# ceres-solver/ceres-solver

Hardware: AMD Instinct MI355X
Metric: LM trust-region steps/sec (linear-solve hot path) + JtJx SpMV HBM GB/s on BAL (higher is better)
Workload: dtype f64; 1 GPU; venice1778-shaped synthetic BAL Jacobian <2,3,9>: 1778 cameras, 993923 points, 5001946 observations, N(0,1) values, seed 38401, camera popularity skew 0.6; solver=ITERATIVE_SCHUR + SCHUR_JACOBI, termination=SUCCESS, parallelism=1 GPU, inputs_resident_in_hbm=True, step_finite=True, jacobian_storage=fp64, camera_accumulators_in_lds=True

## Files before the change

### ceres-solver_amd/csrc/common.h

```cpp
#ifndef CERES_HIP_COMMON_H_
#define CERES_HIP_COMMON_H_

#include <cstdint>
#include <string>
#include <vector>

#include "../../include/ceres_hip.h"

namespace chip {

constexpr int kTile = 64;
constexpr int kMaxGenericBlock = 16;
constexpr int kCamChunk = 512;
constexpr int kPairsPerSlot = 12;
#ifndef CERES_HIP_AB_TILE_ROWS
#define CERES_HIP_AB_TILE_ROWS 12
#endif
constexpr int kTilePitch = CERES_HIP_AB_TILE_ROWS * 64;
constexpr size_t kLdsBytesPerCu = 160 * 1024;
constexpr int kSchurItem = 128;
constexpr int kZUnit = 64;
constexpr int kMaxPointsPerTile = 42;
constexpr int kSlotCamBits = 20;
constexpr int kSlotSpill = 0xFFF;
constexpr int kSlotNoCamera = (1 << kSlotCamBits) - 1;
constexpr int kPipelineMinTilesPerWg = 40;
constexpr int kStagedXMinTilesPerWg = 100;
constexpr int kCamItemLaneMinMean = 384;
constexpr int kCamItemSpread = 8192;
constexpr int kNonTemporalTileMiB = 200;

struct HostStructure {
  int nrb = 0, ncb = 0, nelim = 0, ncells = 0;
  std::vector<int32_t> rsz, rpos, csz, cpos, rptr, ccol, cval;
  int num_rows = 0, num_cols = 0, num_cols_e = 0, num_cols_f = 0, num_row_blocks_e = 0;
  int64_t nnz = 0;
  int64_t values_extent = 0;
  int max_block = 0;
  int det_row = 0, det_e = 0, det_f = 0;
  std::vector<int32_t> tptr, trow, tcell;
  std::vector<int32_t> row_block_of, col_block_of;
  std::vector<int64_t> diag_off_all;
  std::vector<int64_t> diag_off_f;
  std::vector<int64_t> diag_off_e;
  std::vector<int32_t> row_e_block;
  std::vector<int32_t> chunk_start, chunk_size;
  bool chunks_contiguous = true;
};

constexpr int kMaxSharedScalars = 8;
constexpr int kMaxSharedCellsPerRow = 2;
inline bool BalShapeCompiled(int nr, int ne, int nf, int ns) {
  if (nr == 3) return ne == 3 && nf == 3 && ns == 0;
  if (nr == 4) return ne == 4 && ns == 0 && (nf == 2 || nf == 3 || nf == 4);
  if (nr != 2) return false;
  if (ne == 2) return ns == 0 && (nf == 2 || nf == 3 || nf == 4 || nf == 6 || nf == 9);
  if (ne == 4) return ns == 0 && nf >= 2 && nf <= 10;
  if (ne != 3) return false;
  if (ns == 0) return nf >= 2 && nf <= 10;
  return (nf == 6 || nf == 9) && (ns == 4 || ns == 8);
}
inline int BalStripWidthFor(int ns_used) { return ns_used <= 0 ? 0 : (ns_used <= 4 ? 4 : (ns_used <= 8 ? 8 : -1)); }
// ... 102 lines not shown
```

### ceres-solver_amd/csrc/device.h

```cpp
#ifndef CERES_HIP_DEVICE_H_
#define CERES_HIP_DEVICE_H_

#include <hip/hip_runtime.h>

#include <cstdint>

#include "common.h"

namespace chip {

int BalBlockFor(int mode);
constexpr size_t kMaxLdsBytes = 160 * 1024;
constexpr int kVecBlock = 256;
constexpr int kMaxVecGrid = 512;
constexpr int kMaxEvalGrid = 2048;
constexpr int kMaxLsCameraGrid = 4096;

constexpr int kP2pMaxWorld = 8;
constexpr int kP2pChunk = 512;
constexpr int kP2pFlagChunk = 8;
constexpr int kP2pMaxGrid = 256;
struct P2pPeers {
  double* slots[kP2pMaxWorld];
  unsigned long long* flags[kP2pMaxWorld];
// ... 65 lines not shown
  const int32_t* d_pos = nullptr;
  double* D_int_out = nullptr;
  const double* x_e = nullptr;
  const double* x_f = nullptr;
  int flags = 0;
  double* y_e = nullptr;
  const double* D_e = nullptr;
  double lm_radius = 0.0, lm_min = 0.0, lm_max = 0.0;
  double* lm_diag_e = nullptr;
  double* lm_D_e = nullptr;
  double* etei = nullptr;
  double* point_blocks = nullptr;
  const int64_t* pt_diag_off = nullptr;
  double* Mo = nullptr;
  const int32_t* mo_index = nullptr;
  int have_b = 0;
  double* partials = nullptr;
  double* zbuf = nullptr;
  double* strip_sums = nullptr;
  int n_acc = 0;
  const int32_t* xhot_cam = nullptr;
  int n_xhot = 0;
  int x_lds_scalars = 0;
  double* scalar_out = nullptr;
  const double* copy_src = nullptr;
  double* copy_dst = nullptr;
  int copy_n = 0;
  int negate_out = 0;
  int* nonfinite = nullptr;
  const int* run_after_cg = nullptr;
  double* pq_out = nullptr;
  const int* status = nullptr;
  int* clear_flags = nullptr;
  CgTail tail;
};

struct LmFuse {
  double radius = 0.0, min_d = 0.0, max_d = 0.0;
  const double* camsq = nullptr;
  const int32_t* cam_pos = nullptr;
  int cam_base = 0;
  double* diag_f = nullptr;
  double* D_f = nullptr;
};

constexpr int kLossNone = -1, kLossTrivial = 0, kLossHuber = 1, kLossSoftLOne = 2, kLossCauchy = 3, kLossArctan = 4, kLossTolerant = 5,
              kLossTukey = 6;
struct LossParams {
  int32_t type = kLossNone;
  double a = 0.0, b = 0.0, c = 0.0, k = 1.0;
};

struct CamItems {
  const int32_t *cam = nullptr, *begin = nullptr, *end = nullptr;
  int count = 0;
  int64_t observations = 0;
  const double *ev_cam_pack = nullptr, *ev_pt_pack = nullptr;
  const int32_t* ev_pt = nullptr;
  const double2* ev_obs = nullptr;
  LossParams ev_loss;
};
struct CamGather {
  const double* parts = nullptr;
  const int32_t* cam_item_ptr = nullptr;
  const double* D_f = nullptr;
  const int32_t* cam_pos = nullptr;
  int cam_base = 0;
  int want_sq = 0;
  int few = 0;
  const double* extra = nullptr;
  const double* packed = nullptr;
};
struct ZUnits {
  const int32_t *cam = nullptr, *begin = nullptr, *end = nullptr, *shared = nullptr;
  const int32_t* slot = nullptr;
  int first = 0, count = 0;
};

struct FMap {
  const int32_t* cam_pos = nullptr;
  int cam_base = 0, n_cam_scalars = 0;
  int sh_pos[kMaxSharedScalars] = {};
};

struct StripBlocks {
  int count = 0;
  int off[kMaxSharedScalars] = {}, width[kMaxSharedScalars] = {}, pos[kMaxSharedScalars] = {};
  int64_t out[kMaxSharedScalars] = {};
};

struct BalOps {
  int nr, ne, nf, ns, pairs, tile_pitch, cam_part, etei_pitch, b_pairs, mo_pitch, has_f32, has_cg_tail;
  hipError_t (*fused)(int mode, const BalArgs& A, bool lds, int grid, hipStream_t stream);
  bool (*sx_runs_pipelined)(const BalArgs& A);
  hipError_t (*reduce_partials)(const double* partials, int nparts, int n_acc, const FMap& map, const double* D_f, const double* x_f,
                                double* y_f, const int* status, double* pq_out, int* n_pq, hipStream_t stream, const double* sum_in,
                                int n_sum_in, double* sum_out);
  hipError_t (*reduce_exchange)(const double* partials, int nparts, int n_acc, int n_fv, const FMap& map, const double* D_f, const double* x_f,
                                double* y_f, const int* status, double* pq_out, int* n_pq, hipStream_t stream, const double* sum_in,
                                int n_sum_in, double* sum_out, const P2pComm& comm, int grid_cap);
  hipError_t (*stream_probe)(const double2* J, int64_t n_tiles, int grid, double* out, hipStream_t stream);
  hipError_t (*add_f_diagonal)(int n_acc, const FMap& map, const double* D_f, const double* x_f, double* y_f, const int* status,
                               double* pq_out, int* n_pq, hipStream_t stream);
  hipError_t (*pack)(const BalArgs& A, hipStream_t stream);
  hipError_t (*invert)(double* blocks, const int64_t* cam_diag_off, int n_cameras, int* fail_flag, const LmFuse& lm, const CamGather& gather,
                       hipStream_t stream);
  hipError_t (*camera_exchange)(const double* parts, const int32_t* cam_item_ptr, int n_cameras, const double* extra, double* packed,
                                const P2pComm& comm, int grid_cap, hipStream_t stream, bool few );
  hipError_t (*camera_items)(bool schur, const double* values, const CamItems& items, const int32_t* cam_fpos, const int32_t* cam_slot,
                             const double* Mo, double* parts, hipStream_t stream);
  hipError_t (*camera_finish)(const double* parts, const int32_t* cam_item_ptr, const double* D_f, const int32_t* cam_pos, int cam_base,
                              const int64_t* cam_diag_off, double* blocks, double* camsq, int n_cameras, hipStream_t stream, const double* extra,
                              bool few );
  hipError_t (*camera_chunk)(const ZUnits& units, const double* ring, double* acc, const int* status, hipStream_t stream);
  hipError_t (*strip_finish)(const double* parts, int nparts, const StripBlocks& sb, const double* D_f, double* blocks, hipStream_t stream);
};
const BalOps* GetBalOps(int nr, int ne, int nf, int ns);
hipError_t AllowMaxLds(const void* kernel);

constexpr int kGenItem = 128;
constexpr int kGenItemValues = 55;
struct GenItems {
  int count = 0, first_block = 0, nblocks = 0;
  const int32_t *block = nullptr, *t0 = nullptr, *t1 = nullptr;
  const int32_t* block_ptr = nullptr;
  double* scratch = nullptr;
};
struct GenStructure {
  int nrb = 0, ncb = 0, nelim = 0, nrbe = 0, num_rows = 0, num_cols = 0, nce = 0, ncf = 0;
  const int32_t *rsz = nullptr, *rpos = nullptr, *rptr = nullptr, *ccol = nullptr, *cval = nullptr;
  const int32_t *csz = nullptr, *cpos = nullptr;
  const int32_t *tptr = nullptr, *trow = nullptr, *tcell = nullptr;
  const int32_t *tval = nullptr, *trpos = nullptr, *tinfo = nullptr;
  const int32_t *row_block_of = nullptr, *col_block_of = nullptr, *row_e_block = nullptr;
  const int64_t *diag_off_all = nullptr, *diag_off_e = nullptr, *diag_off_f = nullptr;
  const int32_t *chunk_start = nullptr, *chunk_size = nullptr;
  int max_csz_e = 0, max_csz_f = 0, max_csz = 0, max_rsz = 0;
  int lanes_e = 0, lanes_f = 0, lanes_all = 0, lanes_chunk = 0;
  GenItems items;
};
enum GenPart { kAll = 0, kE = 1, kF = 2 };

hipError_t LaunchGenRightMultiply(const GenStructure& G, const double* values, int part, const double* x, double* y,
                                  const int* status, hipStream_t stream);
hipError_t LaunchGenLeftMultiply(const GenStructure& G, const double* values, int part, const double* x, double* y,
                                 const int* status, hipStream_t stream);
hipError_t LaunchGenBlockDiagonal(const GenStructure& G, const double* values, int part, const double* D,
                                  double* blocks, int64_t total_entries, hipStream_t stream);
// ... 92 lines not shown
};
hipError_t LaunchCgnrModelCost(const double* y, const double* g, const double* r, const double* D, int64_t begin, int64_t end,
                               double* partials, int* nparts, hipStream_t stream, double* neg_out = nullptr, int* nonfinite = nullptr,
                               const int* gate = nullptr, const PointPerm& perm = PointPerm());
hipError_t LaunchPermutePoints(const double* in, double* out, const int32_t* pt_pos, int64_t n_e, int64_t n, bool to_internal, hipStream_t stream);
hipError_t LaunchNegateAndCheck(double* x, int64_t n, int* nonfinite, hipStream_t stream);
hipError_t LaunchGenScaleColumns(const GenStructure& G, double* values, const double* scale, hipStream_t stream);
hipError_t LaunchExpandSym(const double* packed, int ne, int pitch, double* dense, const int64_t* pt_diag_off, int n_points, hipStream_t stream);
hipError_t LaunchScatterBlocks9(const double* in, double* out, const int64_t* off, int n_points, hipStream_t stream);

enum CgStatus {
  kCgRunning = 0,
  kCgConvergedZeta = 1,
  kCgConvergedResidual = 2,
  kCgMaxIterations = 3,
  kCgFailRho = 4,
  kCgFailBeta = 5,
  kCgIndefinite = 6,
  kCgFailAlpha = 7,
  kCgZeroRhs = 8,
  kCgInitialResidual = 9,
  kCgSetupFailed = 10,
};
__host__ __device__ inline bool CgStatusAllowsSolution(int st) {
  return st != kCgRunning && st != kCgFailRho && st != kCgFailBeta && st != kCgFailAlpha && st != kCgSetupFailed;
}

struct CgScalars {
  double norm_rhs, tol_r, q_tol;
  double rho, rho_new, beta, pq, alpha, Q0, Q1, zeta, norm_r, norm_p, norm_q;
  int iter, status, min_it, max_it;
  int fail_dir, fail_step;
  double rho_pp[2], Q0_pp[2];
};

struct CgBuffers {
  int64_t n = 0;
  int64_t n_local = 0;
  int grid = 1, grid_e = 0;
  double *x = nullptr, *r = nullptr, *p = nullptr, *z = nullptr;
  const double* rhs = nullptr;
  double* partials = nullptr;
  double* comm = nullptr;
  CgScalars* S = nullptr;
  const int* setup_fail = nullptr;
  const double* pq_parts = nullptr;
  int n_pq = 0;
  const double* pq_extra = nullptr;
};
constexpr int kMaxPqParts = 2048;

hipError_t LaunchCgRhsNorm(const CgBuffers& B, hipStream_t stream);
hipError_t LaunchCgInit(const CgBuffers& B, double q_tol, double r_tol, int min_it, int max_it, hipStream_t stream);
hipError_t LaunchCgPrecondition(const CgBuffers& B, const GenStructure& G, int first_block, int col_begin, int nblocks,
                                int n_local_blocks, const int64_t* diag_off, const double* blocks, hipStream_t stream);
hipError_t LaunchCgDotSlot(const CgBuffers& B, const double* x, const double* y, int slot, hipStream_t stream);
hipError_t LaunchCgInitFromGuess(const CgBuffers& B, const double* tmp, double q_tol, double r_tol, int min_it, int max_it,
                                 hipStream_t stream);
hipError_t LaunchCgDirection(const CgBuffers& B, hipStream_t stream);
hipError_t LaunchCgDotPq(const CgBuffers& B, hipStream_t stream);
hipError_t LaunchCgStep(const CgBuffers& B, int reset, hipStream_t stream);
hipError_t LaunchCgResidualReset(const CgBuffers& B, const double* tmp, hipStream_t stream);
hipError_t LaunchCgFinalize(const CgBuffers& B, hipStream_t stream);
hipError_t LaunchCgUpdate(const CgBuffers& B, const GenStructure& G, int first_block, int col_begin, int nblocks,
                          const int64_t* diag_off, const double* blocks, int reset, int it, int nine_from, hipStream_t stream);
hipError_t LaunchCgBegin(const CgBuffers& B, double q_tol, double r_tol, int min_it, int max_it, hipStream_t stream);
hipError_t LaunchCgFinalizeDirection(const CgBuffers& B, int it, hipStream_t stream);
// ... 148 lines not shown
```

### ceres-solver_amd/csrc/kernels_bal.inc

```
#include <hip/hip_runtime.h>

#include <algorithm>
#include <mutex>
#include <unordered_map>

#include "device.h"
#include "p2p.h"
#ifndef CERES_HIP_NE
#define CERES_HIP_NE 3
#endif
#ifndef CERES_HIP_NR
#define CERES_HIP_NR 2
#endif
#if CERES_HIP_NE == 3 && CERES_HIP_NR == 2
#define CERES_HIP_PIPELINED 1
#else
#define CERES_HIP_PIPELINED 0
#endif
#if CERES_HIP_NR == 2 && CERES_HIP_NE == 3 && CERES_HIP_NF == 9 && CERES_HIP_NS == 0
#define CERES_HIP_IS_BAL_SHAPE 1
#include "robust_loss.h"
#include "snavely.h"
#else
#define CERES_HIP_IS_BAL_SHAPE 0
// ... 707 lines not shown
__device__ __forceinline__ void store_ete_inverse(const BalArgs& A, int pt, const double (&ei)[kTriE]) {
  if (A.etei) {
    double2* q = reinterpret_cast<double2*>(A.etei + int64_t(pt) * kEteiPitch);
#pragma unroll
    for (int j = 0; j < kEteiPitch / 2; ++j) tile_store<2>(q + j, make_double2(ei[2 * j], 2 * j + 1 < kTriE ? ei[(2 * j + 1) % kTriE] : 0.0));
  }
  if (A.point_blocks) {
    double* o = A.point_blocks + (A.pt_diag_off ? A.pt_diag_off[pt] : int64_t(NE * NE) * pt);
#pragma unroll
    for (int i = 0; i < NE; ++i) {
#pragma unroll
      for (int j = 0; j < NE; ++j) o[NE * i + j] = ei[i <= j ? tri_e(i, j) : tri_e(j, i)];
    }
  }
}

__device__ __forceinline__ void slot_point_sums(const Slot& s, double (&r)[kNX]) {
  double a[kTriE], g[NE];
  ete_of(s, a);
  et_times(s.e, s.b, g);
#pragma unroll
  for (int i = 0; i < kTriE; ++i) r[i] = s.valid ? a[i] : 0.0;
#pragma unroll
  for (int j = 0; j < NE; ++j) r[kTriE + j] = s.valid ? g[j] : 0.0;
}
__device__ __forceinline__ void store_point_solution(const BalArgs& A, int po, const double (&v)[NE]) {
  const double sg = A.negate_out ? -1.0 : 1.0;
  double t = 0.0;
#pragma unroll
  for (int j = 0; j < NE; ++j) { A.y_e[po + j] = sg * v[j]; t += v[j]; }
  if (A.negate_out && !isfinite(t)) atomicAdd(A.nonfinite, 1);
}

__device__ __forceinline__ double cost_terms(const double (&m)[NR], const double (&b)[NR], double half) {
  double t = 0.0;
#pragma unroll
  for (int r = 0; r < NR; ++r) t += m[r] * (b[r] + half * m[r]);
  return t;
}

template <bool LDS>
__device__ __forceinline__ void init_apply(const BalArgs& A, const Slot& s, int64_t sl,
                                           const double (&ei)[kTriE], const double (&g)[NE], Ctx& acc) {
  double h[NE], eh[NR], w[NR];
  sym_mul(ei, g, h);
  e_times(s.e, h, eh);
#pragma unroll
  for (int r = 0; r < NR; ++r) w[r] = s.b[r] - eh[r];
  if (A.have_b) scatter_ft<LDS>(A, s, acc, w);
  if (A.Mo && s.valid) {
    double q[NR][NE];
#pragma unroll
    for (int r = 0; r < NR; ++r) {
      double er[NE];
#pragma unroll
      for (int j = 0; j < NE; ++j) er[j] = s.e[r * NE + j];
      sym_mul(ei, er, q[r]);
    }
    double m[kMoPitch];
#pragma unroll
    for (int i = 0; i < kMoPitch; ++i) m[i] = 0.0;
#pragma unroll
    for (int a = 0; a < NR; ++a) {
#pragma unroll
      for (int b = 0; b < NR; ++b) {
        if (b < a) continue;
// ... 14 lines not shown
  double xc[NF];
  double ei[kTriE];
  double xa, xb, da, db;
  double xp[NE], dd[NE];
  int64_t base;
  bool coop;
};

template <int MODE>
__device__ __forceinline__ void load_aux(const BalArgs& A, const Slot& s, int lane, int npts, StreamAux& x) {
  load_xc(A, s.cam, x.xc);
  x.xa = x.xb = x.da = x.db = 0.0;
  x.base = 0;
  x.coop = false;
#pragma unroll
  for (int j = 0; j < NE; ++j) { x.xp[j] = 0.0; x.dd[j] = 0.0; }
  if constexpr (MODE == kSx || MODE == kSpseZ) {
    load_ete_inverse(A, s.pt, x.ei);
  } else if constexpr (MODE == kJtJx) {
    x.coop = CERES_HIP_PIPELINED && A.pt_pos == nullptr && !(A.flags & 1);
    if (x.coop) {
      const int n3 = 3 * npts;
      x.base = 3 * int64_t(__builtin_amdgcn_readfirstlane(s.pt));
      if (lane < n3) { x.xa = A.x_e[x.base + lane]; if (A.D_e) x.da = A.D_e[x.base + lane]; }
      if (n3 > 64 && lane + 64 < n3) { x.xb = A.x_e[x.base + 64 + lane]; if (A.D_e) x.db = A.D_e[x.base + 64 + lane]; }
    } else {
      const int po = pt_off(A, s.pt);
#pragma unroll
      for (int j = 0; j < NE; ++j) { x.xp[j] = A.x_e[po + j]; if (A.D_e) x.dd[j] = A.D_e[po + j]; }
    }
  }
}

template <int MODE, bool LDS>
__device__ __forceinline__ void compute_stream(const BalArgs& A, const Slot& s, int lane, int span, int npts,
                                               const StreamAux& x, Ctx& acc, double& dot) {
  if constexpr (MODE == kSx || MODE == kSpseZ) {
    double v[NE];
    double t[NR];
    f_times(s, acc, x.xc, t);
    double u[NE];
    et_times(s.e, t, u);
    if (!s.valid) {
#pragma unroll
      for (int j = 0; j < NE; ++j) u[j] = 0;
    }
#if !(CERES_HIP_AB_ABLATE & 4)
    seg_allreduce<NE>(u, lane, s.first, s.last, span);
#endif
    sym_mul(x.ei, u, v);
    double ev[NR], z[NR];
    e_times(s.e, v, ev);
#pragma unroll
    for (int r = 0; r < NR; ++r) z[r] = MODE == kSx ? t[r] - ev[r] : ev[r];
    scatter_ft<LDS>(A, s, acc, z);
  } else {
    static_assert(MODE == kJtJx, "streaming modes");
    double xp[NE];
#pragma unroll
    for (int j = 0; j < NE; ++j) xp[j] = x.xp[j];
#if CERES_HIP_PIPELINED
    const int n3 = 3 * npts;
    if (x.coop) {
      const int li = s.valid ? 3 * s.pt - int(x.base) : 0;
      if (n3 <= 64) {
#pragma unroll
        for (int j = 0; j < 3; ++j) xp[j] = shfl_idx(x.xa, li + j);
      } else {
#pragma unroll
        for (int j = 0; j < 3; ++j) {
          const double va = shfl_idx(x.xa, (li + j) & 63), vb = shfl_idx(x.xb, (li + j) & 63);
          xp[j] = (li + j) < 64 ? va : vb;
        }
      }
    }
#endif
    double z[NR];
    f_times(s, acc, x.xc, z);
    {
      double ex[NR];
      e_times(s.e, xp, ex);
#pragma unroll
// ... 154 lines not shown
    scatter_ft<LDS>(A, s, acc, s.b);
    double w[NE];
    et_times(s.e, s.b, w);
    if (!s.valid) {
#pragma unroll
      for (int j = 0; j < NE; ++j) w[j] = 0;
    }
    seg_scan<NE>(w, lane, s.first, span);
    if (s.valid && lane == s.last) {
#pragma unroll
      for (int j = 0; j < NE; ++j) A.y_e[po + j] = w[j];
    }
  } else if constexpr (MODE == kInit || MODE == kEte) {
    double r[kNX];
    slot_point_sums(s, r);
    if constexpr (MODE == kInit) {
      seg_allreduce<kNX>(r, lane, s.first, s.last, span);
    } else {
      double a6[kTriE];
#pragma unroll
      for (int i = 0; i < kTriE; ++i) a6[i] = r[i];
      seg_allreduce<kTriE>(a6, lane, s.first, s.last, span);
#pragma unroll
      for (int i = 0; i < kTriE; ++i) r[i] = a6[i];
    }
    double a[kTriE], ei[kTriE];
#pragma unroll
    for (int i = 0; i < kTriE; ++i) a[i] = r[i];
    add_e_diagonal(A, s.pt, po, a, s.valid && lane == s.last);
    if (!s.valid) set_identity_e(a);
    invert_spd_e(a, ei);
    if (s.valid && lane == s.last) store_ete_inverse(A, s.pt, ei);
    if constexpr (MODE == kInit) {
      double g[NE];
#pragma unroll
      for (int j = 0; j < NE; ++j) g[j] = r[kTriE + j];
      init_apply<LDS>(A, s, sl, ei, g, acc);
    }
  } else if constexpr (MODE == kColNorm) {
    double w[NE];
    e_col_squares(s, w);
    if (!s.valid) {
#pragma unroll
      for (int j = 0; j < NE; ++j) w[j] = 0;
    }
    scatter_f_squares(s, acc);
    seg_scan<NE>(w, lane, s.first, span);
    if (s.valid && lane == s.last) {
#pragma unroll
      for (int j = 0; j < NE; ++j) A.y_e[po + j] = w[j];
    }
  } else if constexpr (MODE == kJx) {
    double xc[NF];
    load_xc(A, s.cam, xc);
    double xe[NE];
#pragma unroll
    for (int j = 0; j < NE; ++j) xe[j] = A.x_e[po + j];
    double m[NR], ex[NR];
    f_times(s, acc, xc, m);
    e_times(s.e, xe, ex);
#pragma unroll
    for (int r = 0; r < NR; ++r) m[r] += ex[r];
    if (s.valid) lane_acc -= cost_terms(m, s.b, 0.5);
  } else if constexpr (MODE == kCgnrInit) {
    double r[kNX];
    slot_point_sums(s, r);
// ... 174 lines not shown
      }
    }
  } else if constexpr (MODE == kInit || MODE == kEte || MODE == kCgnrInit) {
    double r[kNX];
#pragma unroll
    for (int i = 0; i < kNX; ++i) r[i] = 0.0;
    int pt = 0;
    for (int t = 0; t < nt; ++t) {
      load_slot<kCanGather<MODE>, F32>(A, tile + t, lane, s, kWantsB<MODE>);
      if (t == 0) pt = __shfl(s.pt, 0, 64);
      if constexpr (MODE == kCgnrInit) scatter_ft<LDS>(A, s, acc, s.b);
      double q[kNX];
      slot_point_sums(s, q);
#pragma unroll
      for (int i = 0; i < kNX; ++i) r[i] += q[i];
    }
    wave_allreduce<kNX>(r);
    const int po = pt_off(A, pt);
    double a[kTriE], ei[kTriE];
#pragma unroll
    for (int i = 0; i < kTriE; ++i) a[i] = r[i];
    add_e_diagonal(A, pt, po, a, lane == 0);
    invert_spd_e(a, ei);
    if constexpr (MODE == kCgnrInit) {
      if (lane == 0) {
#pragma unroll
        for (int j = 0; j < NE; ++j) A.y_e[po + j] = r[kTriE + j];
        if (A.point_blocks) store_ete_inverse(A, pt, ei);
      }
    } else {
      if (lane == 0) store_ete_inverse(A, pt, ei);
    }
    if constexpr (MODE == kInit) {
      double g[NE];
#pragma unroll
      for (int j = 0; j < NE; ++j) g[j] = r[kTriE + j];
      for (int t = 0; t < nt; ++t) {
        load_slot<false, F32>(A, tile + t, lane, s, true, false);
        const int64_t sl = (tile + t) * kTile + lane;
        init_apply<LDS>(A, s, sl, ei, g, acc);
      }
    }
  }
}

template <int MODE, bool LDS, int BLOCK, bool F32>
__device__ __forceinline__ void fused_long_rounds(const BalArgs& A, int lane, bool grouped, int range, Ctx& acc, double& lane_acc) {
  constexpr int NX = (MODE == kInit || MODE == kEte || MODE == kCgnrInit) ? kNX : NE;
  constexpr int SUBS = BLOCK / 64 / kRoundWaves;
  constexpr bool kTwoPhase = (MODE == kSx || MODE == kSpseZ || MODE == kInit || MODE == kBackSub);
  static_assert(SUBS >= 1, "a workgroup holds at least one round");
  __shared__ double xr[SUBS][kRoundWaves][NX];
  const int wave_all = __builtin_amdgcn_readfirstlane(int(threadIdx.x >> 6));
  const int sub = wave_all / kRoundWaves, wave = wave_all % kRoundWaves;
  const int64_t qe = grouped ? int64_t(A.round_ptr[range + 1]) : int64_t(A.n_seq);
  const int64_t qstride = grouped ? 1 : int64_t(gridDim.x) * SUBS;
  const int64_t q_first = grouped ? int64_t(A.round_ptr[range]) : logical_workgroup() * SUBS;
  int64_t n_iter = 0;
  for (int j = 0; j < (grouped ? 1 : SUBS); ++j) {
    int64_t n = 0;
    if (grouped) { if (q_first < qe) n = A.seq_ptr[qe] - A.seq_ptr[q_first]; }
    else for (int64_t q = q_first + j; q < qe; q += qstride) n += A.seq_ptr[q + 1] - A.seq_ptr[q];
    n_iter = max(n_iter, n);
  }
  int64_t it_q = q_first + (grouped ? 0 : sub);
  bool it_real = grouped ? (sub == 0 && it_q < qe) : it_q < qe;
// ... 96 lines not shown
      }
    } else if (apply_round) {
#pragma unroll
      for (int i = 0; i < NX; ++i) tot[i] = carry[i];
      if (flag & kRoundLast) {
#pragma unroll
        for (int i = 0; i < NX; ++i) carry[i] = 0.0;
      }
      if constexpr (!kTwoPhase) continue;
    }
    if (!active) continue;
    const bool finish = wave == w0 && lane == 0 && !apply_round;
    const bool apply = flag == 0 || apply_round;
    if constexpr (MODE == kColNorm || MODE == kJtb) {
      if (finish) {
#pragma unroll
        for (int j = 0; j < NE; ++j) A.y_e[po + j] = tot[j];
      }
    } else if constexpr (MODE == kJtJx) {
      if (finish) {
#pragma unroll
        for (int j = 0; j < NE; ++j) {
          double d = 0;
          if (A.D_e) { d = A.D_e[po + j]; d = d * d * xp[j]; }
          A.y_e[po + j] = tot[j] + d;
          lane_acc += xp[j] * (tot[j] + d);
        }
      }
    } else if constexpr (MODE == kSx || MODE == kSpseZ || MODE == kBackSub) {
      double ei[kTriE], v[NE], u[NE];
      load_ete_inverse(A, pt, ei);
#pragma unroll
      for (int j = 0; j < NE; ++j) u[j] = tot[j];
      sym_mul(ei, u, v);
      if constexpr (MODE == kBackSub) {
        if (finish) store_point_solution(A, po, v);
        if (!A.scalar_out || !apply) continue;
      } else if (!apply) continue;
      if (apply_round) {
        double xc[NF];
        load_xc(A, s.cam, xc);
        f_times(s, acc, xc, ft);
        if constexpr (MODE == kBackSub) {
#pragma unroll
          for (int r = 0; r < NR; ++r) ft[r] = s.b[r] - ft[r];
        }
      }
      double ev[NR];
      e_times(s.e, v, ev);
      if constexpr (MODE == kBackSub) {
        double m[NR];
#pragma unroll
        for (int r = 0; r < NR; ++r) m[r] = (s.b[r] - ft[r]) + ev[r];
        if (s.valid) lane_acc += cost_terms(m, s.b, -0.5);
      } else {
        double z[NR];
#pragma unroll
        for (int r = 0; r < NR; ++r) z[r] = MODE == kSx ? ft[r] - ev[r] : ev[r];
        scatter_ft<LDS>(A, s, acc, z);
      }
    } else {
      double a[kTriE], ei[kTriE];
#pragma unroll
      for (int i = 0; i < kTriE; ++i) a[i] = tot[i];
      add_e_diagonal(A, pt, po, a, finish);
      invert_spd_e(a, ei);
      if constexpr (MODE == kCgnrInit) {
        if (finish) {
#pragma unroll
          for (int j = 0; j < NE; ++j) A.y_e[po + j] = tot[kTriE + j];
          if (A.point_blocks) store_ete_inverse(A, pt, ei);
        }
      } else {
        if (finish) store_ete_inverse(A, pt, ei);
      }
      if constexpr (MODE == kInit) {
        if (apply) {
          double g[NE];
#pragma unroll
          for (int j = 0; j < NE; ++j) g[j] = tot[kTriE + j];
          init_apply<LDS>(A, s, tile * kTile + lane, ei, g, acc);
        }
      }
    }
  }
}

template <int MODE, bool LDS, int BLOCK, bool F32>
__global__ __launch_bounds__(BLOCK) void bal_fused_kernel(BalArgs A) {
  extern __shared__ double lds_acc[];
  if constexpr (MODE == kInit || MODE == kCgnrInit) {
    if (A.clear_flags && blockIdx.x == 0 && threadIdx.x == 0) { A.clear_flags[0] = 0; A.clear_flags[1] = 0; }
  }
  if (A.status && *A.status != 0) return;
  if (A.run_after_cg && !CgStatusAllowsSolution(*A.run_after_cg)) return;
  constexpr bool kScatters = (MODE == kSx || MODE == kJtJx || MODE == kJtb || MODE == kInit || MODE == kCgnrInit || MODE == kColNorm || MODE == kSpseZ);
  Ctx acc;
  ctx_init(A, acc, nullptr);
  if constexpr (kScatters) {
    acc.lds = lds_acc;
    const int n_acc = LDS ? A.n_acc : NF * A.hyb_rows;
    for (int i = threadIdx.x; i < n_acc; i += BLOCK) acc.lds[i] = 0.0;
    __syncthreads();
  }
  if constexpr (MODE == kBackSub || MODE == kJx) {
    if (A.x_lds_scalars > 0) {
      for (int i = threadIdx.x; i < A.x_lds_scalars; i += BLOCK) lds_acc[i] = A.x_f[cam_off(A, i / NF) + i % NF];
      __syncthreads();
    }
  }
  const int lane = threadIdx.x & 63;
  double lane_acc = 0.0;
  if constexpr (MODE == kBackSub) {
    if (A.copy_dst)
      for (int i = blockIdx.x * BLOCK + threadIdx.x; i < A.copy_n; i += gridDim.x * BLOCK) {
        const double z = A.copy_src[i];
        A.copy_dst[i] = A.negate_out ? -z : z;
        if (A.negate_out && !isfinite(z)) atomicAdd(A.nonfinite, 1);
      }
  }
  const bool grouped = kScatters && !LDS && A.grp_tile_ptr != nullptr;
  const int64_t tile0 = grouped ? A.grp_tile_ptr[blockIdx.x] + (threadIdx.x >> 6) : A.tile_begin + logical_workgroup() * (BLOCK / 64) + (threadIdx.x >> 6);
  const int64_t nwaves = grouped ? BLOCK / 64 : int64_t(gridDim.x) * (BLOCK / 64);
  const int64_t tile_end = grouped ? A.grp_tile_ptr[blockIdx.x + 1] : (A.tile_end > 0 ? A.tile_end : A.n_tiles);
  if constexpr (MODE == kShBlocks) {
    for (int64_t tile = tile0; tile < tile_end; tile += nwaves) {
      const int kind = A.tile_kind[tile];
      const int aux = A.tile_aux[tile];
// ... 208 lines not shown
      const int w = sp + j * ns;
      v[j] = (mine && w < nparts) ? A.partials[int64_t(w) * n + i] : 0.0;
    }
#pragma unroll
    for (int h = kCgTailLoads / 2; h >= 1; h >>= 1) {
#pragma unroll
      for (int j = 0; j < h; ++j) v[j] += v[j + h];
    }
    if (mine) part[idx] = v[0];
  }
  __syncthreads();
  double qv[PER];
  double pq = 0, unused0 = 0, unused1 = 0;
#pragma unroll
  for (int k = 0; k < PER; ++k) {
    const int i = threadIdx.x + k * BLOCK;
    qv[k] = 0.0;
    if (i < n) {
      double q = 0;
      for (int sp = 0; sp < ns; ++sp) q += part[sp * n + i];
      q += dv[k] * dv[k] * pv[k];
      qv[k] = q;
      pq += pv[k] * q;
    }
  }
  sum3(pq, unused0, unused1);
  if (staged) pq = 1.0;
  int fail = staged;
  double alpha = 0;
  if (!fail) {
    if (pq <= 0 || isinf(pq)) fail = kCgIndefinite;
    else { alpha = rho / pq; if (isinf(alpha)) fail = kCgFailAlpha; }
  }
  if (threadIdx.x == 0) { S.pq = pq; S.alpha = alpha; S.rho_new = rho; S.fail_step = fail; }
  if (fail) {
    if (threadIdx.x == 0) S.status = fail;
    return;
  }
  double q1 = 0, rr = 0, rz = 0, rn[PER], zv[PER];
#pragma unroll
  for (int k = 0; k < PER; ++k) {
    const int i = threadIdx.x + k * BLOCK;
    rn[k] = 0.0;
    if (i < n) {
      const double xv = xo[k] + alpha * pv[k];
      const double rv = ro[k] - alpha * qv[k];
      T.x[i] = xv; T.r[i] = rv;
      rn[k] = rv;
      lds[i] = rv;
      q1 -= xv * (bv[k] + rv);
      rr += rv * rv;
    }
  }
  __syncthreads();
#pragma unroll
  for (int k = 0; k < PER; ++k) {
    const int i = threadIdx.x + k * BLOCK;
    zv[k] = 0.0;
    if (i < n) {
      const int c = i / 9;
      double t = 0;
#pragma unroll
      for (int j = 0; j < 9; ++j) t += mrow[k][j] * lds[9 * c + j];
      zv[k] = t;
      T.z[i] = t;
      rz += rn[k] * t;
    }
// ... 3 lines not shown
  const double norm_r = sqrt(rr);
  const double zeta = it * (Q1 - Q0) / Q1;
  int status = kCgRunning;
  if (zeta < q_tol && it >= min_it) status = kCgConvergedZeta;
  else if (norm_r <= tol_r && it >= min_it) status = kCgConvergedResidual;
  else if (it >= max_it) status = kCgMaxIterations;
  int fail_dir = 0;
  double beta = 0.0;
  if (status == kCgRunning) {
    auto zero_or_inf = [](double v) { return v == 0.0 || isinf(v); };
    if (zero_or_inf(rho_next)) fail_dir = kCgFailRho;
    else { beta = rho_next / rho; if (zero_or_inf(beta)) fail_dir = kCgFailBeta; }
    if (!fail_dir) {
#pragma unroll
      for (int k = 0; k < PER; ++k) {
        const int i = threadIdx.x + k * BLOCK;
        if (i < n) T.p[i] = zv[k] + beta * pv[k];
      }
    }
  }
  if (threadIdx.x == 0) {
    S.Q1 = Q1; S.zeta = zeta; S.norm_r = norm_r;
    if (status == kCgConvergedZeta) { S.status = status; return; }
    S.Q0 = Q1;
    S.Q0_pp[(it + 1) & 1] = Q1;
    if (status != kCgRunning) { S.status = status; return; }
    S.rho = rho; S.rho_new = rho_next; S.beta = beta;
    S.rho_pp[(it + 1) & 1] = rho_next;
    S.fail_dir = fail_dir;
    S.iter = it + 1;
  }
}

template <int MODE, bool LDS>
__device__ __forceinline__ void compute_long_round(const BalArgs& A, const Slot& s, int lane, const StreamAux& x, uint32_t word, uint32_t word0,
                                                   int flag, int wave, double (*red)[3], double (&carry)[3], Ctx& acc, double& dot) {
  const bool active = word != kRoundIdle;
  const int w0 = flag ? 0 : (active ? int((word >> 26) & 7u) : wave);
  const int cnt = flag ? int((word0 >> 29) & 7u) + 1 : (active ? int((word >> 29) & 7u) + 1 : 1);
  if constexpr (MODE == kSx || MODE == kSpseZ) {
    double t0, t1;
    f_times(s, acc, x.xc, t0, t1);
    double u[3] = {s.e[0] * t0 + s.e[3] * t1, s.e[1] * t0 + s.e[4] * t1, s.e[2] * t0 + s.e[5] * t1};
    if (!s.valid) { u[0] = u[1] = u[2] = 0; }
    if (!(flag & kRoundApply)) {
      wave_allreduce<3>(u);
      if (lane == 0) { red[wave][0] = u[0]; red[wave][1] = u[1]; red[wave][2] = u[2]; }
    }
    __syncthreads();
    if (flag & kRoundApply) {
      u[0] = carry[0]; u[1] = carry[1]; u[2] = carry[2];
      if (flag & kRoundLast) { carry[0] = carry[1] = carry[2] = 0; }
    } else {
      u[0] = u[1] = u[2] = 0;
      for (int k = 0; k < cnt; ++k) { u[0] += red[w0 + k][0]; u[1] += red[w0 + k][1]; u[2] += red[w0 + k][2]; }
      if (flag & kRoundSum) { carry[0] += u[0]; carry[1] += u[1]; carry[2] += u[2]; return; }
    }
    double v[3];
    sym_mul(x.ei, u, v);
    const double ev0 = s.e[0] * v[0] + s.e[1] * v[1] + s.e[2] * v[2];
    const double ev1 = s.e[3] * v[0] + s.e[4] * v[1] + s.e[5] * v[2];
    scatter_ft<LDS>(A, s, acc, MODE == kSx ? t0 - ev0 : ev0, MODE == kSx ? t1 - ev1 : ev1);
  } else {
    static_assert(MODE == kJtJx, "streaming modes");
    if (flag & kRoundApply) { __syncthreads(); return; }
    const double xp[3] = {shfl_idx(x.xa, 0), shfl_idx(x.xa, 1), shfl_idx(x.xa, 2)};
    double z0, z1;
    f_times(s, acc, x.xc, z0, z1);
    z0 += s.e[0] * xp[0] + s.e[1] * xp[1] + s.e[2] * xp[2];
    z1 += s.e[3] * xp[0] + s.e[4] * xp[1] + s.e[5] * xp[2];
    scatter_ft<LDS>(A, s, acc, z0, z1);
    double w[3] = {s.e[0] * z0 + s.e[3] * z1, s.e[1] * z0 + s.e[4] * z1, s.e[2] * z0 + s.e[5] * z1};
    if (!s.valid) { w[0] = w[1] = w[2] = 0; }
    wave_allreduce<3>(w);
    if (lane == 0) { red[wave][0] = w[0]; red[wave][1] = w[1]; red[wave][2] = w[2]; }
    __syncthreads();
    double t = 0;
    if (lane < 3) {
      for (int k = 0; k < cnt; ++k) t += red[w0 + k][lane];
    }
    bool store = active && wave == w0 && lane < 3;
    if (flag & kRoundSum) {
      const double c = (lane == 0 ? carry[0] : (lane == 1 ? carry[1] : carry[2])) + t;
      if (lane == 0) carry[0] = c; else if (lane == 1) carry[1] = c; else if (lane == 2) carry[2] = c;
      store = store && (flag & kRoundLast);
      t = c;
      if (flag & kRoundLast) { carry[0] = carry[1] = carry[2] = 0; }
    }
    if (store) {
      const double yv = t + x.da * x.da * x.xa;
      A.y_e[x.base + lane] = yv;
      dot += x.xa * yv;
    }
  }
}

template <int MODE, bool LDS, bool NT, bool F32 = false>
__global__ __launch_bounds__(512) void bal_stream_kernel(BalArgs A) {
  constexpr int BLOCK = 512;
  extern __shared__ double lds_acc[];
  if (A.status && *A.status != 0) return;
  Ctx acc;
  ctx_init(A, acc, lds_acc);
  double* const xh = lds_acc + A.n_acc;
  {
    const int n_acc = LDS ? A.n_acc : NF * A.hyb_rows;
    for (int i = threadIdx.x; i < n_acc; i += BLOCK) acc.lds[i] = 0.0;
    if constexpr (LDS) {
      const int nx = NF * A.n_xhot;
      for (int i0 = threadIdx.x; i0 < nx; i0 += 4 * BLOCK) {
        int c[4];
        double v[4];
#pragma unroll
        for (int j = 0; j < 4; ++j) { const int i = i0 + j * BLOCK; c[j] = A.xhot_cam[(i < nx ? i : 0) / NF]; }
#pragma unroll
        for (int j = 0; j < 4; ++j) { const int i = i0 + j * BLOCK; v[j] = A.x_f[A.cam_base + NF * int64_t(c[j]) + (i < nx ? i : 0) % NF]; }
#pragma unroll
        for (int j = 0; j < 4; ++j) { const int i = i0 + j * BLOCK; if (i < nx) xh[i] = v[j]; }
      }
    }
    __syncthreads();
  }
  const int lane = threadIdx.x & 63;
  double dot = 0.0;
  const bool grouped = !LDS && A.grp_tile_ptr != nullptr;
  const int64_t nwaves = grouped ? BLOCK / 64 : int64_t(gridDim.x) * (BLOCK / 64);
  const int wave = __builtin_amdgcn_readfirstlane(int(threadIdx.x >> 6));
  const int range = grouped ? int(blockIdx.x) : 0;
  const int64_t range_end = grouped ? A.grp_tile_ptr[blockIdx.x + 1] : (A.tile_end > 0 ? A.tile_end : A.n_tiles);
  const int64_t long_begin = A.long_behind ? int64_t(A.long_ptr[range]) : range_end;
// ... 19 lines not shown
    issue_idx(A, t1, lane, i2);
    __builtin_amdgcn_sched_barrier(0);
    issue_idx(A, t2, lane, i1);
    __builtin_amdgcn_sched_barrier(0);
    issue_pairs<NT, F32>(A, tile, lane, sa);
    __builtin_amdgcn_sched_barrier(0);
    sa.cam = i0.cam; sa.seg = i0.seg;
    finish_slot(sa, lane, A.tile_pt0[tile]);
    issue_aux<MODE>(A, sa, lane, kind_a == 0 ? aux_a >> 8 : 0, xa);
    __builtin_amdgcn_sched_barrier(0);
    issue_pairs<NT, F32>(A, t1, lane, sb);
    __builtin_amdgcn_sched_barrier(0);
    sb.cam = i2.cam; sb.seg = i2.seg;
    finish_slot(sb, lane, A.tile_pt0[t1]);
    issue_aux<MODE>(A, sb, lane, kind_b == 0 ? aux_b >> 8 : 0, xb);
    __builtin_amdgcn_sched_barrier(0);
    bool more = true;
    auto stage = [&](Slot& c, StreamAux& cx, int ckind, int caux, Slot& f, StreamAux& fx, int& fkind, int& faux) {
      const int64_t far = min(tile + 2 * pstep, last);
      more = tile + pstep < pipe_end;
      fkind = A.tile_kind[far];
      faux = A.tile_aux[far];
      issue_idx(A, min(far + pstep, last), lane, i2);
      __builtin_amdgcn_sched_barrier(0);
      issue_pairs<NT, F32>(A, far, lane, f);
      __builtin_amdgcn_sched_barrier(0);
      f.cam = i1.cam; f.seg = i1.seg;
      finish_slot(f, lane, A.tile_pt0[far]);
      issue_aux<MODE>(A, f, lane, fkind == 0 ? faux >> 8 : 0, fx);
      __builtin_amdgcn_sched_barrier(0);
      if (ckind != 0) c.valid = false;
      widen_slot<F32>(c);
      if constexpr (LDS) take_hot_x(A, c, xh, cx);
      compute_stream<MODE, LDS>(A, c, lane, caux & 0xff, ckind == 0 ? caux >> 8 : 0, cx, acc, dot);
      __builtin_amdgcn_sched_barrier(0);
      i1 = i2;
      tile = min(tile + pstep, last);
    };
    while (true) {
      stage(sa, xa, kind_a, aux_a, sc, xc, kind_c, aux_c);
      if (!more) break;
      stage(sb, xb, kind_b, aux_b, sa, xa, kind_a, aux_a);
      if (!more) break;
      stage(sc, xc, kind_c, aux_c, sb, xb, kind_b, aux_b);
      if (!more) break;
    }
  }
#else
  if (pipe0 < pipe_end) {
    Slot sa, sb;
    StreamAux xa, xb;
    SlotIdx i1, i2;
    int64_t tile = pipe0;
    int kind_a = A.tile_kind[tile], aux_a = A.tile_aux[tile], kind_b = 2, aux_b = 0;
    issue_idx(A, tile, lane, i2);
    __builtin_amdgcn_sched_barrier(0);
    issue_idx(A, min(tile + pstep, last), lane, i1);
    __builtin_amdgcn_sched_barrier(0);
    issue_pairs<NT, F32>(A, tile, lane, sa);
    __builtin_amdgcn_sched_barrier(0);
    sa.cam = i2.cam; sa.seg = i2.seg;
    finish_slot(sa, lane, A.tile_pt0[tile]);
    issue_aux<MODE>(A, sa, lane, kind_a == 0 ? aux_a >> 8 : 0, xa);
    __builtin_amdgcn_sched_barrier(0);
    bool more = true;
    auto stage = [&](Slot& c, StreamAux& cx, int ckind, int caux, Slot& n, StreamAux& nx, int& nkind, int& naux) {
      const int64_t next = min(tile + pstep, last);
      more = tile + pstep < pipe_end;
#if CERES_HIP_AB_ABLATE & 16
      nkind = 0;
      naux = (13 << 8) | 8;
      const int npt0 = int(next) * 13;
#else
      nkind = A.tile_kind[next];
      naux = A.tile_aux[next];
      const int npt0 = A.tile_pt0[next];
#endif
      issue_idx(A, min(next + pstep, last), lane, i2);
      __builtin_amdgcn_sched_barrier(0);
      issue_pairs<NT, F32>(A, next, lane, n);
      __builtin_amdgcn_sched_barrier(0);
      n.cam = i1.cam; n.seg = i1.seg;
      finish_slot(n, lane, npt0);
      issue_aux<MODE>(A, n, lane, nkind == 0 ? naux >> 8 : 0, nx);
      __builtin_amdgcn_sched_barrier(0);
      if (ckind != 0) c.valid = false;
      widen_slot<F32>(c);
      if constexpr (LDS) take_hot_x(A, c, xh, cx);
      compute_stream<MODE, LDS>(A, c, lane, caux & 0xff, ckind == 0 ? caux >> 8 : 0, cx, acc, dot);
      __builtin_amdgcn_sched_barrier(0);
      i1 = i2;
      tile = next;
    };
    while (true) {
      stage(sa, xa, kind_a, aux_a, sb, xb, kind_b, aux_b);
      if (!more) break;
      stage(sb, xb, kind_b, aux_b, sa, xa, kind_a, aux_a);
      if (!more) break;
    }
  }
#endif
  __shared__ double round_red[2][kRoundWaves][3];
  if (A.round_word) {
    const int64_t qe = grouped ? int64_t(A.round_ptr[range + 1]) : int64_t(A.n_seq);
    const int64_t qstride = grouped ? 1 : int64_t(gridDim.x);
    int64_t it_q = grouped ? int64_t(A.round_ptr[range]) : logical_workgroup();
    if (it_q < qe) {
      int64_t it_r = A.seq_ptr[it_q], it_end = A.seq_ptr[grouped ? qe : it_q + 1];
      if (grouped) it_q = qe - 1;
      bool it_real = true;
      auto next_round = [&](bool* real) {
        const int64_t r = it_r;
        *real = it_real;
        if (it_real) {
          if (it_r + 1 < it_end) ++it_r;
          else if (it_q + qstride < qe) { it_q += qstride; it_r = A.seq_ptr[it_q]; it_end = A.seq_ptr[it_q + 1]; }
          else it_real = false;
        }
        return r;
      };
      Slot sa, sb;
      StreamAux xa, xb;
// ... 9 lines not shown
      bool real_c, real_n, real_nn;
      int64_t rc = next_round(&real_c), rn = next_round(&real_n);
      uint32_t wa = word_at(rc), wb = kRoundIdle;
      uint32_t w0a = A.round_word[rc * kRoundWaves], w0b = kRoundIdle;
      int fa = A.round_flag[rc], fb = 0;
      int par = 0;
      {
        const int64_t tile = tile_at(rc, wa);
        issue_idx(A, tile, lane, i2);
        __builtin_amdgcn_sched_barrier(0);
        issue_idx(A, tile_at(rn, word_at(rn)), lane, i1);
        __builtin_amdgcn_sched_barrier(0);
        issue_pairs<NT, F32>(A, tile, lane, sa);
        __builtin_amdgcn_sched_barrier(0);
        finish(sa, i2, tile, wa);
        issue_aux<MODE>(A, sa, lane, 1, xa);
        __builtin_amdgcn_sched_barrier(0);
      }
      auto stage = [&](Slot& c, StreamAux& cx, uint32_t cw, uint32_t cw0, int cf, Slot& n, StreamAux& nx, uint32_t& nw, uint32_t& nw0, int& nf) {
        const int64_t rnn = next_round(&real_nn);
        nw = word_at(rn);
        nw0 = A.round_word[rn * kRoundWaves];
        nf = A.round_flag[rn];
        const int64_t next = int64_t((nw != kRoundIdle ? nw : nw0) & 0x3FFFFFFu);
        issue_idx(A, tile_at(rnn, word_at(rnn)), lane, i2);
        __builtin_amdgcn_sched_barrier(0);
        issue_pairs<NT, F32>(A, next, lane, n);
        __builtin_amdgcn_sched_barrier(0);
        finish(n, i1, next, nw);
        issue_aux<MODE>(A, n, lane, 1, nx);
        __builtin_amdgcn_sched_barrier(0);
        widen_slot<F32>(c);
        if constexpr (LDS) take_hot_x(A, c, xh, cx);
        compute_long_round<MODE, LDS>(A, c, lane, cx, cw, cw0, cf, wave, round_red[par], carry, acc, dot);
        __builtin_amdgcn_sched_barrier(0);
        par ^= 1;
        i1 = i2;
        rc = rn; real_c = real_n;
        rn = rnn; real_n = real_nn;
      };
      while (true) {
        stage(sa, xa, wa, w0a, fa, sb, xb, wb, w0b, fb);
        if (!real_c) break;
        stage(sb, xb, wb, w0b, fb, sa, xa, wa, w0a, fa);
        if (!real_c) break;
      }
    }
  }
  for (int64_t tile = (A.long_behind ? long_begin + wave_first : wave0); tile < range_end; tile += nwaves) {
    if (A.tile_kind[tile] == 1) process_long_point<MODE, LDS, F32>(A, tile, A.tile_aux[tile], lane, acc, dot);
  }
  if (MODE == kJtJx && A.pq_out) {
    __shared__ double red[BLOCK / 64];
#pragma unroll
    for (int m = 32; m >= 1; m >>= 1) dot += __shfl_xor(dot, m, 64);
    if (lane == 0) red[threadIdx.x >> 6] = dot;
    __syncthreads();
    if (threadIdx.x == 0) {
      double t = 0;
      for (int i = 0; i < BLOCK / 64; ++i) t += red[i];
      if (A.pq_accumulate) t += A.pq_out[blockIdx.x];
      A.pq_out[blockIdx.x] = t;
    }
  }
  if constexpr (LDS) {
    flush_shared_sums(A, acc);
    __syncthreads();
// ... 830 lines not shown
  }
}

__global__ __launch_bounds__(1024) void bal_strip_finish_kernel(const double* __restrict__ parts, int nparts, StripBlocks sb,
                                                                const double* __restrict__ D_f, double* __restrict__ blocks) {
  __shared__ double T[16][kTriSX];
  const int lane = threadIdx.x & 63, wv = threadIdx.x >> 6;
  for (int i = lane; i < kTriS; i += 64) {
    double t0 = 0, t1 = 0;
    int w = wv;
    for (; w + 16 < nparts; w += 32) { t0 += parts[int64_t(w) * kTriS + i]; t1 += parts[int64_t(w + 16) * kTriS + i]; }
    if (w < nparts) t0 += parts[int64_t(w) * kTriS + i];
    T[wv][i] = t0 + t1;
  }
  __syncthreads();
  for (int i = threadIdx.x; i < kTriS; i += 1024) {
    double t = T[0][i];
    for (int w = 1; w < 16; ++w) t += T[w][i];
    T[0][i] = t;
  }
  __syncthreads();
  for (int q = 0; q < sb.count; ++q) {
    const int w = sb.width[q], o = sb.off[q];
    for (int e = threadIdx.x; e < w * w; e += 1024) {
      const int a = e / w, b = e - a * w;
      const int lo = o + (a < b ? a : b), hi = o + (a < b ? b : a);
      double v = T[0][lo * (2 * NS + 1 - lo) / 2 + (hi - lo)];
      if (a == b && D_f) { const double d = D_f[sb.pos[q] + a]; v += d * d; }
      blocks[sb.out[q] + e] = v;
    }
  }
}

}

template <int MODE, int BLOCK, bool F32>
static hipError_t launch_fused2(const BalArgs& A, bool lds, int grid, hipStream_t stream) {
  if (lds) {
    const size_t bytes = size_t(A.n_acc) * sizeof(double);
    auto k = bal_fused_kernel<MODE, true, BLOCK, F32>;
    if (hipError_t e = AllowMaxLds(reinterpret_cast<const void*>(k)); e != hipSuccess) return e;
    hipLaunchKernelGGL(k, dim3(grid), dim3(BLOCK), bytes, stream, A);
  } else {
    constexpr bool kScatters = (MODE == kSx || MODE == kJtJx || MODE == kJtb || MODE == kInit || MODE == kCgnrInit || MODE == kColNorm || MODE == kSpseZ);
    const size_t bytes = kScatters ? (size_t(A.hyb_rows) * NF + size_t(BLOCK / 64) * kTile * NF) * sizeof(double)
                                   : ((MODE == kBackSub || MODE == kJx) ? size_t(A.x_lds_scalars) * sizeof(double) : 0);
    auto k = bal_fused_kernel<MODE, false, BLOCK, F32>;
    if (bytes > 0)
      if (hipError_t e = AllowMaxLds(reinterpret_cast<const void*>(k)); e != hipSuccess) return e;
    hipLaunchKernelGGL(k, dim3(grid), dim3(BLOCK), bytes, stream, A);
  }
  return hipGetLastError();
}
template <int MODE, int BLOCK>
static hipError_t launch_fused(const BalArgs& A, bool lds, int grid, hipStream_t stream) {
  if constexpr (kHasF32) {
    if (A.Jf) return launch_fused2<MODE, BLOCK, true>(A, lds, grid, stream);
  } else {
    if (A.Jf) return hipErrorInvalidValue;
  }
  return launch_fused2<MODE, BLOCK, false>(A, lds, grid, stream);
}

#if CERES_HIP_PIPELINED
template <int MODE, bool NT, bool F32 = false>
static hipError_t launch_stream2(const BalArgs& A, bool lds, int grid, hipStream_t stream) {
  if (lds) {
    auto k = bal_stream_kernel<MODE, true, NT, F32>;
    if (hipError_t e = AllowMaxLds(reinterpret_cast<const void*>(k)); e != hipSuccess) return e;
    const size_t tail_bytes = (kHasCgTail && MODE == kSx && A.tail.enabled) ? size_t(512 + kCgTailMax) * sizeof(double) : 0;
    static const size_t static_lds = [&] { hipFuncAttributes fa{}; return hipFuncGetAttributes(&fa, reinterpret_cast<const void*>(k)) == hipSuccess ? size_t(fa.sharedSizeBytes) : size_t(1024); }();
    BalArgs B = A;
    if (size_t(B.n_acc) * sizeof(double) + size_t(B.n_xhot) * NF * sizeof(double) + static_lds > kMaxLdsBytes) B.n_xhot = 0;
    const size_t xhot_bytes = size_t(B.n_xhot) * NF * sizeof(double);
    hipLaunchKernelGGL(k, dim3(grid), dim3(512), size_t(B.n_acc) * sizeof(double) + std::max(tail_bytes, xhot_bytes), stream, B);
  } else {
    auto k = bal_stream_kernel<MODE, false, NT, F32>;
    if (hipError_t e = AllowMaxLds(reinterpret_cast<const void*>(k)); e != hipSuccess) return e;
    hipLaunchKernelGGL(k, dim3(grid), dim3(512), (size_t(A.hyb_rows) * NF + size_t(512 / 64) * kTile * NF) * sizeof(double), stream, A);
  }
  return hipGetLastError();
}
template <int MODE>
static hipError_t launch_stream(const BalArgs& A, bool lds, int grid, hipStream_t stream) {
  if (A.Jf) {
    if constexpr (kHasF32) {
      const bool nt32 = A.n_tiles * int64_t(6 * kTile) * int64_t(sizeof(float4)) > (int64_t(kNonTemporalTileMiB) << 20);
      return nt32 ? launch_stream2<MODE, true, true>(A, lds, grid, stream) : launch_stream2<MODE, false, true>(A, lds, grid, stream);
    } else {
      return hipErrorInvalidValue;
    }
  }
  const bool nt = A.n_tiles * int64_t(kTilePitch) * int64_t(sizeof(double2)) > (int64_t(kNonTemporalTileMiB) << 20);
  return nt ? launch_stream2<MODE, true>(A, lds, grid, stream) : launch_stream2<MODE, false>(A, lds, grid, stream);
}

#endif

static bool UsePipeline() {
  static int v = [] { const char* e = getenv("CERES_HIP_PIPELINE"); return e ? atoi(e) : 1; }();
  return CERES_HIP_PIPELINED && v != 0;
}

static bool F32Pipelined() {
  static int v = [] { const char* e = getenv("CERES_HIP_F32_PIPELINE"); return e ? atoi(e) : 1; }();
  return kHasF32 && v != 0;
}
static bool SxRunsPipelined(const BalArgs& A) { return UsePipeline() && (!A.Jf || F32Pipelined()) && !A.src_values && !A.cam_pos && !(A.flags & 1); }

static hipError_t Fused(int mode, const BalArgs& A0, bool lds, int grid, hipStream_t stream) {
  BalArgs A = A0;
  if ((mode != kBackSub && mode != kJx) || lds) A.x_lds_scalars = 0;
  if ((A.tile_end > 0 ? A.tile_end - A.tile_begin : A.n_tiles) < int64_t(kStagedXMinTilesPerWg) * grid) { A.n_xhot = 0; A.x_lds_scalars = 0; }
  const bool big = BalBlockFor(mode) == 1024;
  const bool few_tiles = (A.tile_end > 0 ? A.tile_end - A.tile_begin : A.n_tiles) < int64_t(kPipelineMinTilesPerWg) * grid && !A.tail.enabled && lds;
  const bool big_s = big && (lds || A.hyb_rows == 0) && !few_tiles;
#if CERES_HIP_PIPELINED
  if (UsePipeline() && !few_tiles && (!A.Jf || F32Pipelined()) && !A.src_values && !A.cam_pos && !(A.flags & 1)) {
    if (mode == kSx) return launch_stream<kSx>(A, lds, grid, stream);
    if (mode == kJtJx && A.D_e && !A.pt_pos) return launch_stream<kJtJx>(A, lds, grid, stream);
    if (mode == kSpseZ) return launch_stream<kSpseZ>(A, lds, grid, stream);
  }
#endif
  switch (mode) {
    case kSx: return big_s ? launch_fused<kSx, 1024>(A, lds, grid, stream) : launch_fused<kSx, 512>(A, lds, grid, stream);
    case kJtJx: return big_s ? launch_fused<kJtJx, 1024>(A, lds, grid, stream) : launch_fused<kJtJx, 512>(A, lds, grid, stream);
// ... 114 lines not shown
  static const int forced = [] { const char* e = getenv("CERES_HIP_CAM_ITEMS_MFMA"); return e ? (atoi(e) != 0 ? 1 : 0) : -1; }();
  const bool mfma = NR == 2 && (forced >= 0 ? forced == 1 : items.observations < int64_t(kCamItemLaneMinMean) * items.count);
  if (mfma) {
#if CERES_HIP_NR == 2
    if (schur) hipLaunchKernelGGL((bal_camera_items_mfma_kernel<true>), grid, dim3(256), 0, stream, values, items, cam_fpos, cam_slot, Mo, parts);
    else hipLaunchKernelGGL((bal_camera_items_mfma_kernel<false>), grid, dim3(256), 0, stream, values, items, cam_fpos, cam_slot, Mo, parts);
#endif
  } else {
    if (schur) hipLaunchKernelGGL((bal_camera_items_kernel<true>), grid, dim3(256), 0, stream, values, items, cam_fpos, cam_slot, Mo, parts);
    else hipLaunchKernelGGL((bal_camera_items_kernel<false>), grid, dim3(256), 0, stream, values, items, cam_fpos, cam_slot, Mo, parts);
  }
  return hipGetLastError();
}

static hipError_t CameraFinish(const double* parts, const int32_t* cam_item_ptr, const double* D_f, const int32_t* cam_pos, int cam_base,
                               const int64_t* cam_diag_off, double* blocks, double* camsq, int n_cameras, hipStream_t stream, const double* extra, bool few) {
  if (n_cameras > 0 && !few) {
    hipLaunchKernelGGL(bal_camera_finish_wide_kernel, dim3(n_cameras), dim3(64 * kInvertGatherWaves), 0, stream, parts, cam_item_ptr, D_f, cam_pos,
                       cam_base, cam_diag_off, blocks, camsq, n_cameras, extra);
    return hipGetLastError();
  }
  if (n_cameras > 0) hipLaunchKernelGGL(bal_camera_finish_kernel, dim3((n_cameras + kPerWave - 1) / kPerWave), dim3(64), 0, stream, parts, cam_item_ptr, D_f, cam_pos,
                                        cam_base, cam_diag_off, blocks, camsq, n_cameras, extra);
  return hipGetLastError();
}

static hipError_t CameraChunk(const ZUnits& units, const double* ring, double* acc, const int* status, hipStream_t stream) {
  if (units.count == 0) return hipSuccess;
  const int waves = (units.count + kPerWave - 1) / kPerWave;
  hipLaunchKernelGGL(bal_camera_chunk_kernel, dim3((waves + 3) / 4), dim3(256), 0, stream, units, ring, acc, status);
  return hipGetLastError();
}

}

#define CERES_HIP_CAT2(a, b) a##b
#define CERES_HIP_CAT(a, b) CERES_HIP_CAT2(a, b)
const BalOps* CERES_HIP_CAT(BalOps_, CERES_HIP_SHAPE)() {
  namespace sh = CERES_HIP_SHAPE;
  static const BalOps ops = {sh::NR, sh::NE, sh::NF, sh::NS, sh::kPairs, sh::kTilePitch, sh::kCamPart, sh::kEteiPitch, sh::kBPairs, sh::kMoPitch, sh::kHasF32 ? 1 : 0, sh::kHasCgTail ? 1 : 0,
                             sh::Fused, sh::SxRunsPipelined, sh::ReducePartials, sh::ReduceExchange, sh::StreamProbe, sh::AddFDiagonal, sh::Pack, sh::Invert, sh::CameraExchange,
                             sh::CameraItems, sh::CameraFinish, sh::CameraChunk, sh::StripFinish};
  return &ops;
}

}
```

### ceres-solver_amd/csrc/kernels_cg.hip

```cpp
#include <hip/hip_runtime.h>

#include <algorithm>

#include "device.h"
#include "p2p.h"

namespace chip {

namespace {

__device__ __forceinline__ double wave_sum(double v) {
#pragma unroll
  for (int m = 32; m >= 1; m >>= 1) v += __shfl_xor(v, m, 64);
  return v;
}

__device__ __forceinline__ double block_sum(double v, double* sh ) {
  v = wave_sum(v);
  __syncthreads();
  if ((threadIdx.x & 63) == 0) sh[threadIdx.x >> 6] = v;
  __syncthreads();
  return (sh[0] + sh[1]) + (sh[2] + sh[3]);
}

// ... 109 lines not shown
    const bool pt = perm.pt_pos && i < perm.n_e;
    const double yi = y[i], d = D ? (pt ? perm.D_e[i] : D[i]) * yi : 0.0;
    v += yi * (g[i] + r[i]) + d * d;
    if (neg_out) { neg_out[pt ? perm.pt_pos[i / 3] + int(i % 3) : i] = -yi; if (!isfinite(yi)) ++bad; }
  }
  if (bad) atomicAdd(nonfinite, bad);
  v = block_sum(v, sh);
  if (threadIdx.x == 0) partials[blockIdx.x] = v;
}

__global__ __launch_bounds__(kVecBlock) void cg_rhs_norm_kernel(CgBuffers B) {
  __shared__ double sh[4];
  double v = 0;
  for (Span s = my_span(B); s.i < s.end; s.i += s.step) v += B.rhs[s.i] * B.rhs[s.i];
  v = block_sum(v, sh);
  if (threadIdx.x == 0) B.partials[blockIdx.x] = v;
}

__global__ __launch_bounds__(kVecBlock) void cg_init_kernel(CgBuffers B, double q_tol, double r_tol, int min_it, int max_it) {
  __shared__ double sh[4];
  const double nn = total_of(B, 0, sh);
  for (Span s = my_span(B); s.i < s.end; s.i += s.step) { B.x[s.i] = 0.0; B.r[s.i] = B.rhs[s.i]; }
  if (blockIdx.x == 0 && threadIdx.x == 0) {
    CgScalars& S = *B.S;
    S.norm_rhs = sqrt(nn);
    S.tol_r = r_tol * S.norm_rhs;
    S.q_tol = q_tol;
    S.rho = 1.0; S.rho_new = 1.0; S.beta = 0; S.pq = 0; S.alpha = 0;
    S.Q0 = 0.0;
    S.Q0_pp[0] = 0.0; S.Q0_pp[1] = 0.0; S.rho_pp[0] = 1.0; S.rho_pp[1] = 1.0;
    S.Q1 = 0; S.zeta = 0; S.norm_r = S.norm_rhs; S.norm_p = 0; S.norm_q = 0;
    S.iter = 1; S.min_it = min_it; S.max_it = max_it;
    S.status = kCgRunning;
    S.fail_dir = 0; S.fail_step = 0;
    if (S.norm_rhs == 0.0) S.status = kCgZeroRhs;
    else if (min_it == 0 && S.norm_r <= S.tol_r) S.status = kCgInitialResidual;
    if (B.setup_fail && *B.setup_fail != 0) S.status = kCgSetupFailed;
  }
}

__global__ __launch_bounds__(kVecBlock) void cg_dot_slot_kernel(CgBuffers B, const double* x, const double* y, int slot) {
  __shared__ double sh[4];
  if (B.S->status != 0) return;
  double v = 0;
  for (Span s = my_span(B); s.i < s.end; s.i += s.step) v += x[s.i] * y[s.i];
  v = block_sum(v, sh);
  if (threadIdx.x == 0) B.partials[slot * kMaxVecGrid + blockIdx.x] = v;
}

__global__ __launch_bounds__(kVecBlock) void cg_init_from_guess_kernel(CgBuffers B, const double* tmp) {
  __shared__ double sh[4];
  double q = 0, rr = 0;
  for (Span s = my_span(B); s.i < s.end; s.i += s.step) {
    const double r = B.rhs[s.i] - tmp[s.i];
    B.r[s.i] = r;
    q -= B.x[s.i] * (B.rhs[s.i] + r);
    rr += r * r;
  }
  q = block_sum(q, sh);
  rr = block_sum(rr, sh);
  if (threadIdx.x == 0) { B.partials[2 * kMaxVecGrid + blockIdx.x] = q; B.partials[3 * kMaxVecGrid + blockIdx.x] = rr; }
}
__global__ __launch_bounds__(kVecBlock) void cg_init_from_guess_finish_kernel(CgBuffers B, double q_tol, double r_tol, int min_it, int max_it) {
  __shared__ double sh[4];
  const double nn = total_of(B, 0, sh);
  const double Q0 = total_of(B, 2, sh);
  const double rr = total_of(B, 3, sh);
  if (threadIdx.x != 0) return;
  CgScalars& S = *B.S;
  S.norm_rhs = sqrt(nn);
  S.tol_r = r_tol * S.norm_rhs;
  S.q_tol = q_tol;
  S.rho = 1.0; S.rho_new = 1.0; S.beta = 0; S.pq = 0; S.alpha = 0;
  S.Q0 = Q0; S.Q1 = 0; S.zeta = 0; S.norm_r = sqrt(rr); S.norm_p = 0; S.norm_q = 0;
  S.Q0_pp[0] = Q0; S.Q0_pp[1] = Q0; S.rho_pp[0] = 1.0; S.rho_pp[1] = 1.0;
  S.iter = 1; S.min_it = min_it; S.max_it = max_it;
  S.status = kCgRunning;
  S.fail_dir = 0; S.fail_step = 0;
  if (S.norm_rhs == 0.0) S.status = kCgZeroRhs;
  else if (min_it == 0 && S.norm_r <= S.tol_r) S.status = kCgInitialResidual;
  if (B.setup_fail && *B.setup_fail != 0) S.status = kCgSetupFailed;
}

template <int N>
__device__ __forceinline__ double precondition_block(const double* __restrict__ m, const double* __restrict__ r, double* __restrict__ z) {
  double rr[N], v = 0;
#pragma unroll
  for (int c = 0; c < N; ++c) rr[c] = r[c];
#pragma unroll
  for (int a = 0; a < N; ++a) {
    double s = 0;
#pragma unroll
    for (int c = 0; c < N; ++c) s += m[a * N + c] * rr[c];
    z[a] = s;
    v += rr[a] * s;
  }
  return v;
}

__global__ __launch_bounds__(kVecBlock) void cg_precondition_kernel(CgBuffers B, GenStructure G, int first_block, int col_begin,
                                                                    int nblocks, int n_local_blocks,
                                                                    const int64_t* diag_off, const double* blocks) {
  __shared__ double sh[4];
  if (B.S->status != 0) return;
  double v = 0;
  if (!blocks) {
    for (Span s = my_span(B); s.i < s.end; s.i += s.step) { const double r = B.r[s.i]; B.z[s.i] = r; v += r * r; }
  } else {
    int64_t q, q_end, q_step;
    if (int(blockIdx.x) < B.grid_e) {
      q = int64_t(blockIdx.x) * kVecBlock + threadIdx.x; q_end = n_local_blocks; q_step = int64_t(B.grid_e) * kVecBlock;
// ... 232 lines not shown
        else if (n == 9) update_block<9, START>(m, alpha, B.p + pos, B.rhs + pos, B.x + pos, B.r + pos, B.z + pos, q1, rr, rz);
        else {
          double rn[kMaxGenericBlock];
          for (int c = 0; c < n; ++c) {
            const double xv = START ? 0.0 : B.x[pos + c] + alpha * B.p[pos + c];
            const double rv = START ? B.rhs[pos + c] : B.r[pos + c] - alpha * B.z[pos + c];
            B.x[pos + c] = xv; B.r[pos + c] = rv; rn[c] = rv;
            q1 -= xv * (B.rhs[pos + c] + rv);
            rr += rv * rv;
          }
          for (int a = 0; a < n; ++a) {
            double t = 0;
            for (int c = 0; c < n; ++c) t += m[a * n + c] * rn[c];
            B.z[pos + a] = t;
            rz += rn[a] * t;
          }
        }
      }
    }
  }
  if (!reset) {
    block_sum3(q1, rr, rz, sh);
    if (threadIdx.x == 0) {
      B.partials[2 * kMaxVecGrid + blockIdx.x] = q1;
      B.partials[3 * kMaxVecGrid + blockIdx.x] = rr;
      B.partials[0 * kMaxVecGrid + blockIdx.x] = rz;
    }
  }
  if (!START && blockIdx.x == 0 && threadIdx.x == 0) {
    S.pq = pq;
    S.alpha = alpha;
    S.rho_new = rho;
    S.fail_step = fail;
  }
}

__global__ __launch_bounds__(kVecBlock) void cg_begin_kernel(CgBuffers B, double q_tol, double r_tol, int min_it, int max_it) {
  __shared__ double sh[12];
  double nn = 0, rho = 0, unused = 0;
  for (int k = B.grid_e + threadIdx.x; k < B.grid; k += kVecBlock) { nn += B.partials[3 * kMaxVecGrid + k]; rho += B.partials[0 * kMaxVecGrid + k]; }
  block_sum3(nn, rho, unused, sh);
  if (B.grid_e > 0) { nn += B.comm[3]; rho += B.comm[0]; }
  const double norm_rhs = sqrt(nn);
  const double tol_r = r_tol * norm_rhs;
  int status = kCgRunning;
  if (norm_rhs == 0.0) status = kCgZeroRhs;
  else if (min_it == 0 && norm_rhs <= tol_r) status = kCgInitialResidual;
  if (B.setup_fail && *B.setup_fail != 0) status = kCgSetupFailed;
  int fail_dir = 0;
  if (status == kCgRunning) {
    if (zero_or_inf(rho)) fail_dir = kCgFailRho;
    else
      for (int64_t i = int64_t(blockIdx.x) * kVecBlock + threadIdx.x; i < B.n; i += int64_t(gridDim.x) * kVecBlock) B.p[i] = B.z[i];
  }
  if (blockIdx.x == 0 && threadIdx.x == 0) {
    CgScalars& S = *B.S;
    S.norm_rhs = norm_rhs; S.tol_r = tol_r; S.q_tol = q_tol;
    S.rho = 1.0; S.rho_new = rho; S.beta = 0; S.pq = 0; S.alpha = 0;
    S.Q0 = 0.0; S.Q1 = 0; S.zeta = 0; S.norm_r = norm_rhs; S.norm_p = 0; S.norm_q = 0;
    S.Q0_pp[0] = 0.0; S.Q0_pp[1] = 0.0; S.rho_pp[0] = 1.0; S.rho_pp[1] = rho;
    S.iter = 1; S.min_it = min_it; S.max_it = max_it;
    S.fail_dir = fail_dir; S.fail_step = 0;
    S.status = status;
  }
}

__global__ __launch_bounds__(kVecBlock) void cg_finalize_direction_kernel(CgBuffers B, int it) {
  __shared__ double sh[12];
  CgScalars& S = *B.S;
  if (S.status != 0) return;
  const int fail = S.fail_step;
  if (fail != 0) {
    if (blockIdx.x == 0 && threadIdx.x == 0) S.status = fail;
    return;
  }
  double Q1 = 0, rr = 0, rho = 0;
  for (int k = B.grid_e + threadIdx.x; k < B.grid; k += kVecBlock) {
    Q1 += B.partials[2 * kMaxVecGrid + k];
    rr += B.partials[3 * kMaxVecGrid + k];
    rho += B.partials[0 * kMaxVecGrid + k];
  }
  block_sum3(Q1, rr, rho, sh);
  if (B.grid_e > 0) { Q1 += B.comm[2]; rr += B.comm[3]; rho += B.comm[0]; }
  const double Q0 = S.Q0_pp[it & 1], rho_prev = S.rho_pp[it & 1];
  const double norm_r = sqrt(rr);
  const double zeta = it * (Q1 - Q0) / Q1;
  int status = kCgRunning;
  if (zeta < S.q_tol && it >= S.min_it) status = kCgConvergedZeta;
  else if (norm_r <= S.tol_r && it >= S.min_it) status = kCgConvergedResidual;
  else if (it >= S.max_it) status = kCgMaxIterations;
  int fail_dir = 0;
  double beta = 0.0;
  if (status == kCgRunning) {
    if (zero_or_inf(rho)) fail_dir = kCgFailRho;
    else { beta = rho / rho_prev; if (zero_or_inf(beta)) fail_dir = kCgFailBeta; }
// ... 282 lines not shown
```

### ceres-solver_amd/csrc/solver.hip

```cpp
#include <hip/hip_runtime.h>
#include <rccl/rccl.h>

#include <exception>
#include <new>
#include <algorithm>
#include <chrono>
#include <climits>
#include <cmath>
#include <complex>
#include <cstdarg>
#include <cstdio>
#include <cstring>
#include <functional>
#include <limits>
#include <memory>
#include <mutex>
#include <numeric>
#include <sstream>
#include <string>
#include <type_traits>
#include <vector>

#include "device.h"

// ... 41 lines not shown
  uint32_t* d_slot_seg = nullptr;
  int32_t *d_tile_kind = nullptr, *d_tile_aux = nullptr, *d_pt_pos = nullptr, *d_cam_pos = nullptr;
  int32_t *d_cam_ptr = nullptr, *d_cam_fpos = nullptr, *d_cam_slot = nullptr;
  int32_t *d_tile_zbase = nullptr, *d_grp_tile_ptr = nullptr;
  unsigned int* d_cg_ticket = nullptr;
  bool cg_tail_enabled = [] { const char* e = getenv("CERES_HIP_CG_TAIL"); return !e || atoi(e) != 0; }();
  bool cam_exchange_few = false;
  bool cam_items_few = false;
  int32_t *d_long_ptr = nullptr, *d_round_ptr = nullptr, *d_seq_ptr = nullptr, *d_round_flag = nullptr;
  uint32_t* d_round_word = nullptr;
  int32_t* d_mo_index = nullptr;
  CamItems cam_items;
  int32_t* d_cam_item_ptr = nullptr;
  double* d_cam_parts = nullptr;
  double* d_cam_packed = nullptr;
  ZUnits zunits;
  int chunk_grid = 0;
  double *lm_diag = nullptr, *lm_D = nullptr, *scalar_partials = nullptr;
  int* d_nonfinite = nullptr;
  bool clear_flags_pending = false;
  bool fail_flag_clean = false, nonfinite_clean = false;
  bool have_lm_diag = false;
  bool lm_want_model_cost = false;
  bool lm_skip_model_cost = false;
  bool lm_negate_in_solve = false;
  bool lm_negated = false;
  bool lm_cgnr_copy_pending = false;
  bool speculate = true;
  bool lm_speculate = false;
  bool gate_on_cg_status = false;
  bool spec_tail_done = false;
  int spec_cgnr_parts = 0;
  int backsub_cost_parts = 0;
  bool lm_fuse_active = false;
  ceres_hip_lm_options lm_opts{};
  double* d_camsq = nullptr;
  int64_t *d_pt_diag_off = nullptr, *d_cam_diag_off = nullptr;
  int64_t* d_pt_eoff = nullptr;
  double2 *d_J = nullptr, *d_bt = nullptr;
  float4* d_Jf = nullptr;
  double *d_Mo = nullptr, *d_partials = nullptr, *d_global_acc = nullptr;
  int32_t* d_xhot_cam = nullptr;
  double* d_zbuf = nullptr;
  bool merged_layout = false;
  bool merge_step_reduce = false;
  bool rhs_reduce_pending = false;
  double* cgnr_rhs_tail = nullptr;
  GenStructure GR;
  int rem_rows = 0, rem_b0 = 0;
  double *rem_tmp = nullptr, *rem_blocks = nullptr, *rem_b = nullptr;
  int32_t* d_rem_row_map = nullptr;
  int32_t* d_cam_block = nullptr;
  bool rem_blocks_valid = false;
  int bal_flags = 0;
  bool lds_mode = false;
  int fused_grid = 0;
  bool cgnr_internal = false;
  double* D_int = nullptr;
  bool D_int_valid = false;
  bool precond_internal = false;

  double *own_values = nullptr, *own_b = nullptr, *own_D = nullptr, *own_x = nullptr;
  const double *values = nullptr, *b = nullptr, *D = nullptr;

  double* etei = nullptr;
  double* rhs_f = nullptr;
// ... 400 lines not shown
      HIP_TRY(s, s->ops->camera_chunk(U, s->d_zbuf, s->d_global_acc, status, s->stream));
    }
  }
  const double* parts = s->lds_mode ? s->d_partials : s->d_global_acc;
  const int nparts = s->lds_mode ? s->fused_grid : 1;
  int n_second = 0;
  if (s->world <= 1 && has_remainder(s)) {
    HIP_TRY(s, s->ops->reduce_partials(parts, nparts, n9, map, nullptr, nullptr, y_f, status, nullptr, nullptr, s->stream, nullptr, 0, nullptr));
    TRY(add_remainder(s, mode, x_f, y_f, status));
    HIP_TRY(s, s->ops->add_f_diagonal(n9, map, D_f, x_f, y_f, status, pq ? pq + n_first : nullptr, &n_second, s->stream));
  } else if (s->world <= 1) {
    HIP_TRY(s, s->ops->reduce_partials(parts, nparts, n9, map, D_f, x_f, y_f, status, pq ? pq + n_first : nullptr, &n_second, s->stream, nullptr, 0, nullptr));
  } else if (!defer_allreduce && reduction_exchanges(s)) {
    const bool pack = pq && pq_extra && n_first > 0;
    HIP_TRY(s, s->ops->reduce_exchange(parts, nparts, n9, nfv, map, D_f, x_f, y_f, status, pq, &n_second, s->stream,
                                       pack ? pq + kMaxVecGrid : nullptr, n_first, pack ? y_f + nfv : nullptr, next_exchange(s), s->p2p_grid_cap));
    if (pack) *pq_extra = y_f + nfv;
    else if (n_first > 0) { pq = nullptr; n_second = 0; }
    n_first = 0;
  } else {
    const bool pack = pq && pq_extra && n_first > 0;
    HIP_TRY(s, s->ops->reduce_partials(parts, nparts, n9, map, nullptr, nullptr, y_f, status, nullptr, nullptr, s->stream,
                                       pack ? pq : nullptr, n_first, pack ? y_f + nfv : nullptr));
    TRY(add_remainder(s, mode, x_f, y_f, status));
    if (!defer_allreduce) TRY(allreduce(s, y_f, size_t(nfv) + (pack ? 1 : 0)));
    if (pack) { *pq_extra = y_f + nfv; n_first = 0; }
    else if (n_first > 0) { pq = nullptr; n_first = 0; }
    HIP_TRY(s, s->ops->add_f_diagonal(n9, map, D_f, x_f, y_f, status, pq, &n_second, s->stream));
  }
  if (n_pq) *n_pq = n_first + n_second;
  return 0;
}

int op_sx(ceres_hip_solver* s, const double* x, double* y, const int* status, double* pq = nullptr, int* n_pq = nullptr) {
  const HostStructure& h = s->hs;
  if (n_pq) *n_pq = 0;
  if (s->path == CERES_HIP_PATH_BAL) {
    TRY(ensure_packed(s));
    BalArgs A = bal_args(s);
    A.x_f = x;
    return bal_scatter(s, kBalSx, A, x, y, true, status, pq, n_pq);
  }
  const double* v = s->values;
  hipStream_t st = s->stream;
  const int first_free_row = h.num_row_blocks_e < h.nrb ? h.rpos[h.num_row_blocks_e] : h.num_rows;
  const hipError_t fe = LaunchGenChunkSx(s->G, v, s->etei, x, s->tmp_rows, status, st);
  hipError_t pe = hipSuccess;
  if (fe == hipSuccess) {
    if (first_free_row < h.num_rows) {
      HIP_TRY(s, hipMemsetAsync(s->tmp_rows + first_free_row, 0, sizeof(double) * (h.num_rows - first_free_row), st));
      HIP_TRY(s, LaunchGenRightMultiplyFrom(s->G, v, kF, first_free_row, x, s->tmp_rows, status, st));
    }
  } else if (fe != hipErrorNotSupported) {
    HIP_TRY(s, fe);
  } else {
    HIP_TRY(s, hipMemsetAsync(s->tmp_rows, 0, sizeof(double) * h.num_rows, st));
    HIP_TRY(s, LaunchGenRightMultiply(s->G, v, kF, x, s->tmp_rows, status, st));
    pe = LaunchGenChunkProject(s->G, v, s->etei, s->tmp_rows, 1, nullptr, status, st);
  }
  if (pe == hipErrorNotSupported) {
    HIP_TRY(s, hipMemsetAsync(s->tmp_e, 0, sizeof(double) * std::max(1, h.num_cols_e), st));
    HIP_TRY(s, LaunchGenLeftMultiply(s->G, v, kE, s->tmp_rows, s->tmp_e, status, st));
    HIP_TRY(s, hipMemsetAsync(s->tmp_e2, 0, sizeof(double) * std::max(1, h.num_cols_e), st));
    HIP_TRY(s, LaunchGenBlockDiagonalApply(s->G, 0, h.nelim, s->G.diag_off_e, s->etei, s->tmp_e, s->tmp_e2, status, st));
    HIP_TRY(s, LaunchAxpby(-1.0, s->tmp_e2, 0.0, s->tmp_e2, s->tmp_e2, h.num_cols_e, st));
    HIP_TRY(s, LaunchGenRightMultiply(s->G, v, kE, s->tmp_e2, s->tmp_rows, status, st));
  } else {
    HIP_TRY(s, pe);
  }
  const double* D_f = s->D ? s->D + h.num_cols_e : nullptr;
  if (s->world <= 1) {
    HIP_TRY(s, LaunchSquareScale(D_f, x, y, h.num_cols_f, status, st));
    HIP_TRY(s, LaunchGenLeftMultiply(s->G, v, kF, s->tmp_rows, y, status, st));
// ... 21 lines not shown
  }
  HIP_TRY(s, hipMemsetAsync(s->tmp_rows, 0, sizeof(double) * h.num_rows, st));
  HIP_TRY(s, LaunchGenRightMultiply(s->G, s->values, kAll, x, s->tmp_rows, status, st));
  HIP_TRY(s, LaunchSquareScale(nullptr, x, y, h.num_cols, status, st));
  HIP_TRY(s, LaunchGenLeftMultiply(s->G, s->values, kAll, s->tmp_rows, y, status, st));
  if (s->world > 1) TRY(allreduce(s, y + h.num_cols_e, size_t(h.num_cols_f)));
  HIP_TRY(s, LaunchAddSquareScale(s->D, x, y, h.num_cols, status, st));
  return 0;
}

int op_jtb(ceres_hip_solver* s, double* y) {
  const HostStructure& h = s->hs;
  hipStream_t st = s->stream;
  if (!s->have_b) return fail(s, CERES_HIP_E_INVALID, "no residual vector loaded");
  if (s->path == CERES_HIP_PATH_BAL) {
    BalArgs A = bal_args(s);
    A.y_e = y;
    PackGuard g = use_gather_if_unpacked(s, A);
    return g.commit(bal_scatter(s, kBalJtb, A, nullptr, y + h.num_cols_e, false, nullptr));
  }
  HIP_TRY(s, hipMemsetAsync(y, 0, sizeof(double) * h.num_cols, st));
  HIP_TRY(s, LaunchGenLeftMultiply(s->G, s->values, kAll, s->b, y, nullptr, st));
  if (s->world > 1) TRY(allreduce(s, y + h.num_cols_e, size_t(h.num_cols_f)));
  return 0;
}

int op_schur_init(ceres_hip_solver* s, bool want_Mo) {
  const HostStructure& h = s->hs;
  hipStream_t st = s->stream;
  if (s->path == CERES_HIP_PATH_BAL) {
    BalArgs A = bal_args(s);
    A.D_e = s->D;
    A.Mo = want_Mo ? s->d_Mo : nullptr;
    if (s->clear_flags_pending) { A.clear_flags = s->d_nonfinite; s->clear_flags_pending = false; }
    PackGuard g = use_gather_if_unpacked(s, A);
    if (s->have_b) {
      const bool defer = s->world > 1 && s->merge_step_reduce && s->merged_layout;
      TRY(g.commit(bal_scatter(s, kBalInit, A, nullptr, s->rhs_f, false, nullptr, nullptr, nullptr, nullptr, defer)));
      s->rhs_reduce_pending = defer;
      return 0;
    }
    HIP_TRY(s, s->ops->fused(kBalInit, A, s->lds_mode, s->lds_mode ? s->fused_grid : s->chunk_grid, st));
    return g.commit(0);
  }
  HIP_TRY(s, LaunchGenBlockDiagonal(s->G, s->values, kE, s->D, s->etei, h.diag_off_e.back(), st));
  HIP_TRY(s, hipMemsetAsync(s->d_fail_flag, 0, sizeof(int), st));
  HIP_TRY(s, LaunchGenInvertBlocks(s->G, 0, h.nelim, s->G.diag_off_e, s->etei, s->d_fail_flag, st));
  if (!s->have_b) return 0;
  HIP_TRY(s, hipMemcpyAsync(s->tmp_rows, s->b, sizeof(double) * h.num_rows, hipMemcpyDeviceToDevice, st));
  const hipError_t pe = LaunchGenChunkProject(s->G, s->values, s->etei, s->tmp_rows, 1, nullptr, nullptr, st);
  if (pe == hipErrorNotSupported) {
    HIP_TRY(s, hipMemsetAsync(s->tmp_e, 0, sizeof(double) * std::max(1, h.num_cols_e), st));
    HIP_TRY(s, LaunchGenLeftMultiply(s->G, s->values, kE, s->b, s->tmp_e, nullptr, st));
    HIP_TRY(s, hipMemsetAsync(s->tmp_e2, 0, sizeof(double) * std::max(1, h.num_cols_e), st));
    HIP_TRY(s, LaunchGenBlockDiagonalApply(s->G, 0, h.nelim, s->G.diag_off_e, s->etei, s->tmp_e, s->tmp_e2, nullptr, st));
    HIP_TRY(s, hipMemsetAsync(s->tmp_rows, 0, sizeof(double) * h.num_rows, st));
    HIP_TRY(s, LaunchGenRightMultiply(s->G, s->values, kE, s->tmp_e2, s->tmp_rows, nullptr, st));
    HIP_TRY(s, LaunchAxpby(1.0, s->b, -1.0, s->tmp_rows, s->tmp_rows, h.num_rows, st));
  } else {
    HIP_TRY(s, pe);
  }
  HIP_TRY(s, hipMemsetAsync(s->rhs_f, 0, sizeof(double) * std::max(1, h.num_cols_f), st));
  HIP_TRY(s, LaunchGenLeftMultiply(s->G, s->values, kF, s->tmp_rows, s->rhs_f, nullptr, st));
  TRY(allreduce(s, s->rhs_f, size_t(h.num_cols_f)));
  return 0;
}

int op_back_substitute(ceres_hip_solver* s, const double* z, double* x) {
  const HostStructure& h = s->hs;
  hipStream_t st = s->stream;
  if (!s->have_b) return fail(s, CERES_HIP_E_INVALID, "no residual vector loaded");
  if (s->path == CERES_HIP_PATH_BAL) {
    TRY(ensure_packed(s));
    BalArgs A = bal_args(s);
    A.x_f = z; A.y_e = x;
    s->backsub_cost_parts = 0;
    if (s->lm_want_model_cost && z != nullptr) { A.scalar_out = s->scalar_partials; s->backsub_cost_parts = s->fused_grid; }
    if (h.num_cols_f > 0 && z != nullptr) { A.copy_src = z; A.copy_dst = x + h.num_cols_e; A.copy_n = h.num_cols_f; }
    if (s->gate_on_cg_status) A.run_after_cg = &s->cg.S->status;
    if (s->lm_negate_in_solve && z != nullptr) {
      if (!s->nonfinite_clean) HIP_TRY(s, hipMemsetAsync(s->d_nonfinite, 0, sizeof(int), st));
      s->nonfinite_clean = false;
      A.negate_out = 1; A.nonfinite = s->d_nonfinite;
      s->lm_negated = true;
    }
    HIP_TRY(s, s->ops->fused(kBalBackSub, A, false, s->fused_grid, st));
    if (s->backsub_cost_parts > 0 && has_remainder(s)) {
      TRY(rem_model_cost(s, z, 0, s->scalar_partials + s->backsub_cost_parts));
      ++s->backsub_cost_parts;
    }
    return 0;
  } else {
    HIP_TRY(s, hipMemsetAsync(s->tmp_rows, 0, sizeof(double) * h.num_rows, st));
    if (h.num_cols_f > 0) HIP_TRY(s, LaunchGenRightMultiply(s->G, s->values, kF, z, s->tmp_rows, nullptr, st));
    HIP_TRY(s, LaunchAxpby(1.0, s->b, -1.0, s->tmp_rows, s->tmp_rows, h.num_rows, st));
    HIP_TRY(s, hipMemsetAsync(x, 0, sizeof(double) * h.num_cols, st));
    const hipError_t pe = LaunchGenChunkProject(s->G, s->values, s->etei, s->tmp_rows, 0, x, nullptr, st);
    if (pe == hipErrorNotSupported) {
      HIP_TRY(s, hipMemsetAsync(s->tmp_e, 0, sizeof(double) * std::max(1, h.num_cols_e), st));
      HIP_TRY(s, LaunchGenLeftMultiply(s->G, s->values, kE, s->tmp_rows, s->tmp_e, nullptr, st));
      HIP_TRY(s, LaunchGenBlockDiagonalApply(s->G, 0, h.nelim, s->G.diag_off_e, s->etei, s->tmp_e, x, nullptr, st));
    } else {
      HIP_TRY(s, pe);
    }
  }
  if (h.num_cols_f > 0)
    HIP_TRY(s, hipMemcpyAsync(x + h.num_cols_e, z, sizeof(double) * h.num_cols_f, hipMemcpyDeviceToDevice, st));
  return 0;
}

int invert_shared_blocks(ceres_hip_solver* s, double* out) {
  const BalPlan& P = s->plan;
// ... 265 lines not shown
    A.y_e = out;
    PackGuard g = use_gather_if_unpacked(s, A);
    return g.commit(bal_scatter(s, kBalColNorm, A, nullptr, out + h.num_cols_e, false, nullptr));
  }
  TRY(require_caller_values(s, "SquaredColumnNorm with the cameras' sums outside LDS"));
  HIP_TRY(s, LaunchGenSquaredColumnNorm(s->G, s->values, out, s->stream));
  if (s->world > 1) TRY(allreduce(s, out + h.num_cols_e, size_t(h.num_cols_f)));
  return 0;
}

int enqueue_model_cost_change(ceres_hip_solver* s, const double* x, const double** dev_parts, int* nparts) {
  const HostStructure& h = s->hs;
  hipStream_t st = s->stream;
  if (s->path == CERES_HIP_PATH_BAL) {
    TRY(ensure_packed(s));
    BalArgs A = bal_args(s);
    A.x_e = x; A.x_f = x + h.num_cols_e;
    A.scalar_out = s->scalar_partials;
    *nparts = std::min(s->fused_grid, kMaxVecGrid - 1);
    *dev_parts = s->scalar_partials;
    HIP_TRY(s, s->ops->fused(kBalJx, A, false, *nparts, st));
    if (has_remainder(s)) { TRY(rem_model_cost(s, x + h.num_cols_e, 1, s->scalar_partials + *nparts)); ++*nparts; }
    return 0;
  }
  HIP_TRY(s, hipMemsetAsync(s->tmp_rows, 0, sizeof(double) * h.num_rows, st));
  HIP_TRY(s, LaunchGenRightMultiply(s->G, s->values, kAll, x, s->tmp_rows, nullptr, st));
  double* t2 = s->scratch_vec + h.num_cols;
  HIP_TRY(s, LaunchAxpby(-1.0, s->b, -0.5, s->tmp_rows, t2, h.num_rows, st));
  HIP_TRY(s, LaunchDot(s->tmp_rows, t2, h.num_rows, s->scalar_partials, s->cg.comm, st));
  *nparts = 1;
  *dev_parts = s->cg.comm;
  return 0;
}
struct CgSpec {
  int64_t n = 0;
  int64_t n_local = 0;
  std::function<int(const double*, double*)> apply;
  std::function<int(const double*, double*, double*, int*, const double**)> apply_dot;
  std::function<int()> before_poll;
  std::function<int(int)> iteration;
  bool shard_fused = false;
  std::function<int(const double*, double*)> precondition;
  bool x0_nonzero = false;
  const double* rhs = nullptr;
  int first_block = 0, col_begin = 0, nblocks = 0, n_local_blocks = 0;
  const int64_t* diag_off = nullptr;
  const double* blocks = nullptr;
  const int* setup_fail = nullptr;
};

void fill_summary(const CgScalars& S, int device_status, ceres_hip_summary* out) {
  out->residual_norm = -1.0;
  out->num_iterations = S.iter;
  char* m = out->message;
  const size_t n = sizeof(out->message);
  switch (device_status) {
    case kCgZeroRhs:
      out->termination_type = CERES_HIP_SUCCESS; out->num_iterations = 0;
      snprintf(m, n, "Convergence. |b| = 0."); break;
    case kCgInitialResidual:
      out->termination_type = CERES_HIP_SUCCESS; out->num_iterations = 0;
      snprintf(m, n, "Convergence. |r| = %e <= %e.", S.norm_r, S.tol_r); break;
    case kCgConvergedZeta:
      out->termination_type = CERES_HIP_SUCCESS;
      snprintf(m, n, "Iteration: %d Convergence: zeta = %e < %e. |r| = %e", S.iter, S.zeta, S.q_tol, S.norm_r); break;
    case kCgConvergedResidual:
// ... 90 lines not shown
    B.grid = B.grid_e + grid_for(B.n - B.n_local, kMaxVecGrid / 2);
  } else {
    B.grid_e = 0;
    B.grid = grid_for(B.n, kMaxVecGrid);
  }
  const int min_it = s->opt.min_num_iterations, max_it = s->opt.max_num_iterations;
  const int reset_period = std::max(1, s->opt.residual_reset_period);
  const int* status = &B.S->status;
  const bool adaptive = s->opt.cg_check_interval <= 0;
  int interval = adaptive ? std::max(2, std::min(s->last_cg_iterations, 64)) : s->opt.cg_check_interval;
  bool first_batch = true;

  const bool fused = s->cg_fused && !spec.precondition && (B.grid_e == 0 || spec.shard_fused);
  const bool fused_start = fused && !spec.x0_nonzero;
  if (fused_start) {
    HIP_TRY(s, LaunchCgUpdate(B, s->G, spec.first_block, spec.col_begin, spec.nblocks, spec.diag_off, spec.blocks, 0, 0,
                              s->nine_wide_from - spec.first_block, st));
    TRY(collapse_and_reduce(s, 0, 4));
    HIP_TRY(s, LaunchCgBegin(B, q_tol, r_tol, min_it, max_it, st));
  } else {
  HIP_TRY(s, LaunchCgRhsNorm(B, st));
  TRY(collapse_and_reduce(s, 0, 1));
  if (spec.x0_nonzero) {
    HIP_TRY(s, hipMemsetAsync(&B.S->status, 0, sizeof(int), st));
    TRY(spec.apply(B.x, B.z));
    HIP_TRY(s, LaunchCgInitFromGuess(B, B.z, q_tol, r_tol, min_it, max_it, st));
  } else {
    HIP_TRY(s, LaunchCgInit(B, q_tol, r_tol, min_it, max_it, st));
  }
  }
  s->h_scalars->status = kCgRunning;
  s->timing.operator_applications = 0;
  int it = 1;
  auto precondition = [&]() -> int {
    if (spec.precondition) {
      TRY(spec.precondition(B.r, B.z));
      HIP_TRY(s, LaunchCgDotSlot(B, B.r, B.z, 0, st));
    } else {
      HIP_TRY(s, LaunchCgPrecondition(B, s->G, spec.first_block, spec.col_begin, spec.nblocks,
                                      B.grid_e > 0 ? spec.n_local_blocks : 0, spec.diag_off, spec.blocks, st));
    }
    return 0;
  };
  if (fused && !fused_start) {
    TRY(precondition());
    TRY(collapse_and_reduce(s, 0, 1));
    HIP_TRY(s, LaunchCgDirection(B, st));
  }
  while (s->h_scalars->status == kCgRunning) {
    const int batch_end = std::min(max_it, it + interval - 1);
    for (; it <= batch_end; ++it) {
      const int reset = (it % reset_period == 0) ? 1 : 0;
      if (fused && spec.iteration && !reset) {
        const int done = spec.iteration(it);
        if (done < 0) return CERES_HIP_E_HIP;
        if (done > 0) { ++s->timing.operator_applications; continue; }
      }
      if (fused) {
        int n_pq = 0;
        const double* extra = nullptr;
        if (spec.apply_dot) TRY(spec.apply_dot(B.p, B.z, s->cg_pq_parts, &n_pq, &extra));
        else TRY(spec.apply(B.p, B.z));
        B.pq_extra = extra;
        if (n_pq > 0) { B.pq_parts = s->cg_pq_parts; B.n_pq = n_pq; }
        else if (B.grid_e > 0) return fail(s, CERES_HIP_E_INVALID, "internal: sharded fused CG needs p.q from the operator");
        else {
          HIP_TRY(s, LaunchCgDotPq(B, st));
          B.pq_parts = B.partials + kMaxVecGrid; B.n_pq = B.grid;
        }
        HIP_TRY(s, LaunchCgUpdate(B, s->G, spec.first_block, spec.col_begin, spec.nblocks, spec.diag_off, spec.blocks, reset, it,
                                  s->nine_wide_from - spec.first_block, st));
        ++s->timing.operator_applications;
        if (reset) {
          TRY(spec.apply(B.x, B.z));
          HIP_TRY(s, LaunchCgResidualReset(B, B.z, st));
          TRY(precondition());
          ++s->timing.operator_applications;
        }
        TRY(collapse_and_reduce(s, 0, 4));
        HIP_TRY(s, LaunchCgFinalizeDirection(B, it, st));
        continue;
      }
      TRY(precondition());
      TRY(collapse_and_reduce(s, 0, 1));
      HIP_TRY(s, LaunchCgDirection(B, st));
      TRY(spec.apply(B.p, B.z));
      HIP_TRY(s, LaunchCgDotPq(B, st));
      TRY(collapse_and_reduce(s, 1, 1));
      HIP_TRY(s, LaunchCgStep(B, reset, st));
      ++s->timing.operator_applications;
      if (reset) {
        TRY(spec.apply(B.x, B.z));
        HIP_TRY(s, LaunchCgResidualReset(B, B.z, st));
        ++s->timing.operator_applications;
      }
      TRY(collapse_and_reduce(s, 2, 2));
      HIP_TRY(s, LaunchCgFinalize(B, st));
    }
    if (spec.before_poll) TRY(spec.before_poll());
    TRY(poll_scalars(s));
    if (adaptive) { interval = first_batch ? 2 : std::min(16, interval * 2); first_batch = false; }
    if (it > max_it && s->h_scalars->status == kCgRunning)
      return fail(s, CERES_HIP_E_INVALID, "CG did not terminate after max_num_iterations (device status 0)");
  }
  (void)status;
  if (s->h_scalars->status == kCgZeroRhs && spec.x0_nonzero) HIP_TRY(s, hipMemsetAsync(B.x, 0, sizeof(double) * B.n, st));
  fill_summary(*s->h_scalars, s->h_scalars->status, summary);
  s->last_cg_iterations = summary->num_iterations;
  return 0;
}

int check_factorization(ceres_hip_solver* s, bool* failed) {
  int flag = 0;
  HIP_TRY(s, hipMemcpyAsync(&flag, s->d_fail_flag, sizeof(int), hipMemcpyDeviceToHost, s->stream));
  HIP_TRY(s, hipStreamSynchronize(s->stream));
  if (s->world > 1) {
    double v = flag != 0 ? 1.0 : 0.0;
    if (!s->d_verdict) TRY(dev_alloc(s, &s->d_verdict, 1));
    HIP_TRY(s, hipMemcpyAsync(s->d_verdict, &v, sizeof(double), hipMemcpyHostToDevice, s->stream));
    TRY(allreduce(s, s->d_verdict, 1));
    HIP_TRY(s, hipMemcpyAsync(&v, s->d_verdict, sizeof(double), hipMemcpyDeviceToHost, s->stream));
    HIP_TRY(s, hipStreamSynchronize(s->stream));
    TRY(check_comm_error(s));
    flag = !(v == 0.0);
  }
  *failed = flag != 0;
  return 0;
}

int cluster_jacobi_eliminate(ceres_hip_solver* s) {
  hipStream_t st = s->stream;
// ... 320 lines not shown
          return 0;
        }
      }
      s->precond_valid = true;
    }
    if (s->rhs_reduce_pending) {
      TRY(allreduce(s, s->rhs_f, size_t(h.num_cols_f)));
      s->rhs_reduce_pending = false;
    }
    TRY(rec(s, 4));
    CgSpec spec;
    spec.rhs = s->rhs_f;
    spec.n = h.num_cols_f;
    spec.n_local = 0;
    const int* status = &s->cg.S->status;
    spec.apply = [s, status](const double* in, double* out) { return op_sx(s, in, out, status); };
    if (s->path == CERES_HIP_PATH_BAL)
      spec.apply_dot = [s, status](const double* in, double* out, double* pq, int* n_pq, const double** extra) {
        *extra = nullptr;
        return op_sx(s, in, out, status, pq, n_pq);
      };
    spec.first_block = h.nelim;
    spec.nblocks = h.ncb - h.nelim;
    spec.col_begin = h.num_cols_e;
    spec.diag_off = s->G.diag_off_f;
    spec.blocks = (pre == CERES_HIP_IDENTITY || spse_pre || cluster_pre) ? nullptr : s->precond;
    if (cg_tail_possible(s) && spec.blocks) {
      spec.iteration = [s, status](int it) -> int {
        if (ensure_packed(s)) return -1;
        BalArgs A = bal_args(s);
        if (!s->ops->sx_runs_pipelined(A)) return 0;
        CgBuffers& B = s->cg;
        A.x_f = B.p;
        A.status = status;
        A.tail.enabled = 1; A.tail.it = it; A.tail.ticket = s->d_cg_ticket;
        A.tail.x = B.x; A.tail.r = B.r; A.tail.p = B.p; A.tail.z = B.z; A.tail.rhs = B.rhs;
        A.tail.blocks = s->precond; A.tail.D_f = s->D ? s->D + s->hs.num_cols_e : nullptr; A.tail.S = B.S;
        if (hipError_t e = s->ops->fused(kBalSx, A, true, s->fused_grid, s->stream); e != hipSuccess) {
          fail(s, CERES_HIP_E_HIP, "S.x + CG iteration launch: %s", hipGetErrorString(e));
          return -1;
        }
        return 1;
      };
    }
    if (defer_check && spec.blocks) spec.setup_fail = s->d_fail_flag;
    if (spse_pre)
      spec.precondition = [s, spse_iters, status](const double* in, double* out) { return op_spse_apply(s, in, out, spse_iters, 0.0, status); };
    if (cluster_pre)
      spec.precondition = [s, status](const double* in, double* out) { return op_cluster_jacobi_apply(s, in, out, status); };
    if (s->opt.use_spse_initialization) {
      TRY(op_spse_apply(s, s->rhs_f, s->cg.x, spse_iters, s->opt.spse_tolerance, nullptr));
      spec.x0_nonzero = true;
    }
    s->spec_tail_done = false;
    if (s->lm_speculate && s->path == CERES_HIP_PATH_BAL && h.num_cols_f > 0) {
      spec.before_poll = [s, x]() {
        s->gate_on_cg_status = true;
        const int rc = op_back_substitute(s, s->cg.x, x);
        s->gate_on_cg_status = false;
        if (rc) return rc;
        if (s->world > 1) {
          if (s->mailbox && s->d_h_pinned) {
            s->tail_mailbox_seq = ++s->mailbox_seq;
            HIP_TRY(s, LaunchCollectScalarsExchange(s->d_nonfinite, s->scalar_partials, s->backsub_cost_parts, s->scalar_partials + kSumsOffset,
                                                    next_exchange(s), s->stream, s->scalar_partials, kReadbackDoubles, s->d_h_pinned, s->d_stamp,
                                                    s->tail_mailbox_seq));
          } else {
            HIP_TRY(s, LaunchCollectScalarsExchange(s->d_nonfinite, s->scalar_partials, s->backsub_cost_parts, s->scalar_partials + kSumsOffset,
                                                    next_exchange(s), s->stream));
          }
        }
        s->spec_tail_done = true;
        return 0;
      };
    }
    TRY(run_cg(s, spec, q_tol, r_tol, summary));
    TRY(rec(s, 5));
    if (summary->termination_type != CERES_HIP_FAILURE && summary->termination_type != CERES_HIP_FATAL_ERROR && !s->spec_tail_done)
      TRY(op_back_substitute(s, s->cg.x, x));
    TRY(rec(s, 6));
    return 0;
  }
  const int pre = s->opt.preconditioner_type;
  TRY(rec(s, 3));
  if (s->path == CERES_HIP_PATH_BAL) {
    s->merge_step_reduce = s->world > 1 && !camera_blocks_exchange(s);
    s->D_int_valid = false;
    const int rc_setup = op_cgnr_setup_bal(s, pre == CERES_HIP_JACOBI, s->cg_rhs, s->precond);
    s->merge_step_reduce = false;
    TRY(rc_setup);
    TRY(ensure_D_int(s));
  } else {
    if (pre == CERES_HIP_JACOBI) TRY(op_preconditioner(s, pre, s->precond, true));
    TRY(op_jtb(s, s->cg_rhs));
  }
  const bool defer_check = s->path == CERES_HIP_PATH_BAL;
  if (pre == CERES_HIP_JACOBI) {
    if (!defer_check) {
      bool bad = false;
      TRY(check_factorization(s, &bad));
      if (bad) {
        summary->termination_type = CERES_HIP_FAILURE;
        snprintf(summary->message, sizeof(summary->message), "Preconditioner update failed.");
        return 0;
      }
    }
    s->precond_valid = true;
  }
  TRY(rec(s, 4));
  CgSpec spec;
  spec.n = h.num_cols;
  spec.n_local = h.num_cols_e;
// ... 346 lines not shown
    C = ClusterLayout();
    C.num_clusters = num_clusters; C.n = h.num_cols_f;
    int32_t* q32 = nullptr; int64_t* q64 = nullptr;
    TRY(dev_upload(s, &q32, L.perm)); C.perm = q32;
    TRY(dev_upload(s, &q32, L.cl_off)); C.cl_off = q32;
    TRY(dev_upload(s, &q32, L.block_cluster)); C.block_cluster = q32;
    TRY(dev_upload(s, &q32, L.block_loc)); C.block_loc = q32;
    TRY(dev_upload(s, &q64, L.mat_off)); C.mat_off = q64;
    std::vector<int32_t> small;
    s->cluster_large.clear();
    for (int k = 0; k < num_clusters; ++k) {
      const int dim = L.cl_off[k + 1] - L.cl_off[k];
      if (dim <= kClusterLdsDim) { small.push_back(k); C.small_max_dim = std::max(C.small_max_dim, dim); }
      else s->cluster_large.push_back(k);
    }
    C.n_small = int(small.size());
    TRY(dev_upload(s, &q32, small)); C.small_list = q32;
    TRY(dev_alloc(s, &s->d_Cblk, std::max<size_t>(1, size_t(s->cluster_storage.num_values()))));
    TRY(dev_alloc(s, &s->d_Cmat, std::max<size_t>(1, size_t(L.mat_off.back()))));
    TRY(dev_alloc(s, &s->d_Cvec, std::max<size_t>(1, size_t(h.num_cols_f))));
    if (s->path == CERES_HIP_PATH_BAL) TRY(dev_alloc(s, &s->etei_dense, size_t(h.diag_off_e.back())));
  }
  const int64_t cg_n = is_schur(s) ? h.num_cols_f : h.num_cols;
  TRY(dev_alloc(s, &s->cg.x, size_t(cg_n)));
  TRY(dev_alloc(s, &s->cg.r, size_t(cg_n)));
  TRY(dev_alloc(s, &s->cg.p, size_t(cg_n)));
  TRY(dev_alloc(s, &s->cg.z, size_t(cg_n) + 8));
  TRY(dev_alloc(s, &s->cg_rhs, size_t(cg_n)));
  TRY(dev_alloc(s, &s->cg.partials, size_t(4 * kMaxVecGrid)));
  TRY(dev_alloc(s, &s->cg.comm, 4));
  TRY(dev_alloc(s, &s->cg_pq_parts, size_t(kMaxPqParts)));
  { const char* e = getenv("CERES_HIP_CG_FUSED"); s->cg_fused = !(e && atoi(e) == 0); }
  { const char* e = getenv("CERES_HIP_SPECULATE"); s->speculate = !(e && atoi(e) == 0); }
  s->cg.S = reinterpret_cast<CgScalars*>(s->scalar_partials + kScalarsOffset);
  HIP_TRY(s, hipMemsetAsync(s->cg.S, 0, sizeof(CgScalars), s->stream));
  TRY(dev_alloc(s, &s->precond, size_t(is_schur(s) ? h.diag_off_f.back() : h.diag_off_all.back()) + 2 * size_t(h.num_cols_f)));
  if (is_schur(s)) {
    TRY(dev_alloc(s, &s->ftf_inv, size_t(h.diag_off_f.back())));
    TRY(dev_alloc(s, &s->spse_a, size_t(h.num_cols_f)));
    TRY(dev_alloc(s, &s->spse_b, size_t(h.num_cols_f)));
  }

  if (s->path == CERES_HIP_PATH_BAL) {
    BalPlan& P = s->plan;
    TRY(dev_upload(s, &s->d_slot_epos, P.slot_epos));
    TRY(dev_upload(s, &s->d_slot_fpos, P.slot_fpos));
    TRY(dev_upload(s, &s->d_slot_bpos, P.slot_bpos));
    if (P.ns > 0) {
      for (int q = 0; q < kMaxSharedCellsPerRow; ++q) { TRY(dev_upload(s, &s->d_slot_hpos[q], P.slot_hpos[q])); TRY(dev_upload(s, &s->d_slot_hdesc[q], P.slot_hdesc[q])); }
      std::vector<int64_t> cfo(P.n_cameras);
      for (int c = 0; c < P.n_cameras; ++c) cfo[c] = h.diag_off_f[P.cam_block[c] - h.nelim];
      TRY(dev_upload(s, &s->d_cam_foff, cfo));
    }
    TRY(dev_upload(s, &s->d_slot_cam, P.slot_word));
    if (!P.xhot_cam.empty()) TRY(dev_upload(s, &s->d_xhot_cam, P.xhot_cam));
    TRY(dev_upload(s, &s->d_tile_pt0, P.tile_pt0));
    TRY(dev_upload(s, &s->d_slot_seg, P.slot_seg));
    TRY(dev_upload(s, &s->d_tile_kind, P.tile_kind));
    TRY(dev_alloc(s, &s->d_cg_ticket, 1));
    HIP_TRY(s, hipMemsetAsync(s->d_cg_ticket, 0, sizeof(unsigned int), s->stream));
    TRY(dev_upload(s, &s->d_long_ptr, P.long_ptr));
    TRY(dev_upload(s, &s->d_round_ptr, P.round_ptr));
    s->d_round_word = nullptr;
    if (!P.round_word.empty()) {
      TRY(dev_upload(s, &s->d_round_word, P.round_word));
      TRY(dev_upload(s, &s->d_seq_ptr, P.seq_ptr));
// ... 33 lines not shown
      std::vector<int64_t> peo(P.n_points);
      for (int p = 0; p < P.n_points; ++p) peo[p] = h.diag_off_e[P.pt_block[p]];
      TRY(dev_upload(s, &s->d_pt_eoff, peo));
    }
    const size_t n_slots = size_t(P.n_tiles) * kTile;
    if (s->opt.jacobian_storage == 1) TRY(dev_alloc(s, &s->d_Jf, n_slots * 6));
    else TRY(dev_alloc(s, &s->d_J, size_t(P.n_tiles) * s->ops->tile_pitch));
    TRY(dev_alloc(s, &s->d_bt, n_slots * s->ops->b_pairs));
    TRY(dev_alloc(s, &s->d_Mo, size_t(s->ops->mo_pitch) * n_slots));
    TRY(dev_alloc(s, &s->etei, size_t(P.n_points) * s->ops->etei_pitch));
    const size_t n9 = size_t(P.nf) * P.n_cameras + size_t(P.ns);
    s->lds_mode = P.cameras_in_lds;
    s->fused_grid = s->lds_mode ? s->num_cus : std::min(s->num_cus * 4, 2 * kMaxVecGrid - 2);
    { const char* e = getenv("CERES_HIP_FUSED_GRID"); if (e && atoi(e) > 0 && s->lds_mode) s->fused_grid = std::min(s->fused_grid, atoi(e)); }
    const int64_t tiles_per_wg = 512 / kTile;
    s->fused_grid = int(std::max<int64_t>(1, std::min<int64_t>(s->fused_grid, (P.n_tiles + tiles_per_wg - 1) / tiles_per_wg)));
    s->fused_grid = std::min(s->fused_grid, kMaxPqParts - kMaxVecGrid);
    TRY(dev_alloc(s, &s->d_partials, s->lds_mode ? size_t(s->fused_grid) * n9 : 1));
    TRY(dev_alloc(s, &s->d_global_acc, n9));
    TRY(dev_alloc(s, &s->d_zbuf, s->lds_mode ? size_t(1) : size_t(P.z_ring_rows) * P.nf));
    if (!P.mo_index.empty()) TRY(dev_upload(s, &s->d_mo_index, P.mo_index));
    if (!s->lds_mode) {
      TRY(dev_upload(s, &s->d_tile_zbase, P.tile_zbase));
      if (P.hybrid) TRY(dev_upload(s, &s->d_grp_tile_ptr, P.grp_tile_ptr));
      int32_t *uc = nullptr, *ub = nullptr, *ue = nullptr, *us = nullptr, *zs = nullptr;
      TRY(dev_upload(s, &uc, P.zu_cam)); TRY(dev_upload(s, &ub, P.zu_begin)); TRY(dev_upload(s, &ue, P.zu_end));
      TRY(dev_upload(s, &us, P.zu_shared)); TRY(dev_upload(s, &zs, P.zc_slot));
      s->zunits.cam = uc; s->zunits.begin = ub; s->zunits.end = ue; s->zunits.shared = us; s->zunits.slot = zs;
      int64_t chunk_tiles = 0;
      for (size_t k = 0; k + 1 < P.zc_tile_ptr.size(); ++k) chunk_tiles = std::max<int64_t>(chunk_tiles, P.zc_tile_ptr[k + 1] - P.zc_tile_ptr[k]);
      s->chunk_grid = P.hybrid ? P.hyb_groups : int(std::max<int64_t>(1, std::min<int64_t>(s->num_cus, (chunk_tiles + 15) / 16)));
    }
    TRY(dev_alloc(s, &s->d_camsq, n9));
    if (P.ns > 0) TRY(dev_alloc(s, &s->d_strip_parts, size_t(s->fused_grid) * size_t(P.ns * (P.ns + 1) / 2)));
    if (s->cgnr_internal) TRY(dev_alloc(s, &s->D_int, size_t(h.num_cols_e)));
    if (s->world > 1 && (is_schur(s) ? (P.cameras_contiguous && P.cam_base == 0) : P.caller_contiguous) && int64_t(n9) == int64_t(h.num_cols_f)) {
      s->merged_layout = true;
      if (is_schur(s)) {
        s->rhs_f = s->precond + h.diag_off_f.back();
        s->d_camsq = s->rhs_f + n9;
      } else {
        s->cgnr_rhs_tail = s->precond + h.diag_off_all.back();
      }
    }
    if (P.n_rem_rows > 0) {
      const int nr = P.n_rem_rows;
      GenStructure& R = s->GR;
      R = s->G;
      R.items = GenItems();
      R.lanes_e = R.lanes_f = R.lanes_all = R.lanes_chunk = 0;
      R.nrb = nr; R.nrbe = 0;
      std::vector<int32_t> rsz(nr), rpos(nr), rptr(nr + 1, 0), ccol, cval, rbo, row_map, tptr(h.ncb + 1, 0), trow, tcell;
      std::vector<int32_t> rem_of(h.nrb, -1), cell_of(h.rptr[h.nrb], -1);
      int nscal = 0;
      for (int i = 0; i < nr; ++i) {
        const int ro = P.rem_list[i];
        rem_of[ro] = i;
        rsz[i] = h.rsz[ro];
        rpos[i] = nscal;
        for (int r = 0; r < h.rsz[ro]; ++r) { rbo.push_back(i); row_map.push_back(h.rpos[ro] + r); }
        nscal += h.rsz[ro];
        for (int k = h.rptr[ro]; k < h.rptr[ro + 1]; ++k) { cell_of[k] = int32_t(ccol.size()); ccol.push_back(h.ccol[k]); cval.push_back(h.cval[k]); }
        rptr[i + 1] = int32_t(ccol.size());
      }
      s->rem_rows = nscal;
      R.num_rows = nscal;
// ... 527 lines not shown
```

### ceres-solver_amd/csrc/solver_debug.inc

```

int ceres_hip_debug_staged_x_plan(const ceres_hip_block_structure* bs, int32_t num_eliminate_blocks, int64_t counts[4], int32_t* staged_cam,
                                  int32_t* slot_word, int64_t staged_capacity, int64_t slot_capacity) {
  try {
  if (!bs || !counts) return CERES_HIP_E_INVALID;
  HostStructure h;
  if (!AnalyzeStructure(*bs, num_eliminate_blocks, &h).empty()) return CERES_HIP_E_INVALID;
  BalPlan P;
  HybridRequest hyb;
  hyb.groups = 256;
  hyb.rows = 0;
  hyb.lds_bytes = int64_t(kMaxLdsBytes) - 512;
  BuildBalPlan(h, num_eliminate_blocks > 0 ? kReorderAlways : kReorderIfContiguous, hyb, &P);
  if (!P.eligible) return CERES_HIP_E_UNSUPPORTED;
  counts[0] = P.n_tiles; counts[1] = P.n_cameras; counts[2] = int64_t(P.xhot_cam.size());
  counts[3] = int64_t((size_t(P.nf) * P.n_cameras + size_t(P.ns)) * sizeof(double));
  if (staged_capacity >= int64_t(P.xhot_cam.size()) && staged_cam)
    for (size_t r = 0; r < P.xhot_cam.size(); ++r) staged_cam[r] = P.xhot_cam[r];
  const int64_t n_slots = P.n_tiles * kTile;
  if (slot_capacity >= n_slots && slot_word)
    for (int64_t i = 0; i < n_slots; ++i) slot_word[i] = P.slot_cam[i] < 0 ? -1 : P.slot_word[i];
  return 0;
  } catch (...) { return CERES_HIP_E_INVALID; }
}

int ceres_hip_debug_cluster_cameras(const ceres_hip_block_structure* bs, int32_t num_eliminate_blocks, int32_t visibility_clustering_type,
                                    int32_t* membership, int32_t* num_clusters) {
  try {
  if (!bs || !membership || !num_clusters) return CERES_HIP_E_INVALID;
  HostStructure h;
  if (!AnalyzeStructure(*bs, num_eliminate_blocks, &h).empty()) return CERES_HIP_E_INVALID;
  if (num_eliminate_blocks <= 0 || !h.chunks_contiguous) return CERES_HIP_E_INVALID;
  std::vector<int32_t> m;
// ... 148 lines not shown
```

### ceres-solver_amd/hip_solver.py

```python
from __future__ import annotations

import ctypes
import os
from ctypes import POINTER, byref, c_char, c_char_p, c_double, c_int32, c_int64, c_uint8, c_uint32, c_void_p
from dataclasses import dataclass, field
from typing import List, Optional

import numpy as np

from .block_structure import BlockStructure, CBlockStructure

DENSE_SCHUR, ITERATIVE_SCHUR, CGNR = 3, 5, 6
IDENTITY, JACOBI, SCHUR_JACOBI, SCHUR_POWER_SERIES_EXPANSION, CLUSTER_JACOBI = 0, 1, 2, 3, 4
CANONICAL_VIEWS, SINGLE_LINKAGE = 0, 1
SUCCESS, NO_CONVERGENCE, FAILURE, FATAL_ERROR = 0, 1, 2, 3
PATH_GENERIC, PATH_BAL = 0, 1
E_INVALID, E_UNSUPPORTED, E_HIP, E_COMM, E_NODEVICE = -1, -2, -3, -4, -5
TERMINATION_NAMES = {0: "SUCCESS", 1: "NO_CONVERGENCE", 2: "FAILURE", 3: "FATAL_ERROR"}
UNIQUE_ID_BYTES = 128
IPC_HANDLE_BYTES = 64

(TIMED_JTJX, TIMED_SX, TIMED_SCHUR_INIT, TIMED_SCHUR_JACOBI, TIMED_BACK_SUBSTITUTE, TIMED_PACK, TIMED_BLOCK_JACOBI, TIMED_COPY,
 TIMED_READ_STREAM, TIMED_CGNR_SETUP, TIMED_MODEL_COST, TIMED_JACOBIAN_GRAM, TIMED_CLUSTER_ELIMINATE, TIMED_CLUSTER_FACTOR,
 TIMED_CLUSTER_APPLY) = range(1, 16)
# ... 33 lines not shown
    _fields_ = [("upload_ms", c_double), ("pack_ms", c_double), ("setup_ms", c_double), ("preconditioner_ms", c_double),
                ("cg_ms", c_double), ("back_substitute_ms", c_double), ("download_ms", c_double), ("total_ms", c_double),
                ("operator_applications", c_int32), ("reserved", c_int32)]


class CLmOptions(ctypes.Structure):
    _fields_ = [("radius", c_double), ("min_diagonal", c_double), ("max_diagonal", c_double), ("eta", c_double),
                ("reuse_diagonal", c_int32), ("values_unchanged", c_int32)]


class CLmResult(ctypes.Structure):
    _fields_ = [("linear_solver", CSummary), ("model_cost_change", c_double), ("step_is_finite", c_int32),
                ("reserved", c_int32)]


_DP = POINTER(c_double)
ABI_VERSION = 2

ABI = [
    ("ceres_hip_abi_version", c_int32, []),
    ("ceres_hip_device_count", c_int32, []),
    ("ceres_hip_create", c_void_p, [POINTER(COptions)]),
    ("ceres_hip_destroy", None, [c_void_p]),
    ("ceres_hip_last_error", c_char_p, [c_void_p]),
    ("ceres_hip_set_structure", c_int32, [c_void_p, POINTER(CBlockStructure)]),
    ("ceres_hip_get_info", c_int32, [c_void_p, POINTER(CInfo)]),
    ("ceres_hip_comm_get_unique_id", c_int32, [POINTER(c_uint8)]),
    ("ceres_hip_comm_init", c_int32, [c_void_p, POINTER(c_uint8), c_int32, c_int32]),
    ("ceres_hip_comm_p2p_prepare", c_int32, [c_void_p, c_int32, c_int32, c_int64, POINTER(c_uint8)]),
    ("ceres_hip_comm_p2p_connect", c_int32, [c_void_p, POINTER(c_uint8)]),
    ("ceres_hip_comm_p2p_selftest", c_int32, [c_void_p]),
    ("ceres_hip_comm_p2p_disable", c_int32, [c_void_p]),
    ("ceres_hip_debug_allreduce_timing", c_int32, [c_void_p, c_int64, c_int32, _DP]),
    ("ceres_hip_solve", c_int32, [c_void_p, _DP, _DP, _DP, c_double, c_double, _DP, POINTER(CSummary)]),
    ("ceres_hip_solve_device", c_int32, [c_void_p, c_void_p, c_void_p, c_void_p, c_double, c_double, c_void_p, POINTER(CSummary)]),
    ("ceres_hip_solve_unchanged_values", c_int32, [c_void_p, _DP, c_double, c_double, _DP, POINTER(CSummary)]),
    ("ceres_hip_load", c_int32, [c_void_p, _DP, _DP, _DP]),
    ("ceres_hip_load_device", c_int32, [c_void_p, c_void_p, c_void_p, c_void_p]),
    ("ceres_hip_op_right_multiply", c_int32, [c_void_p, _DP, _DP]),
    ("ceres_hip_op_left_multiply", c_int32, [c_void_p, _DP, _DP]),
    ("ceres_hip_op_right_multiply_e", c_int32, [c_void_p, _DP, _DP]),
    ("ceres_hip_op_right_multiply_f", c_int32, [c_void_p, _DP, _DP]),
    ("ceres_hip_op_left_multiply_e", c_int32, [c_void_p, _DP, _DP]),
    ("ceres_hip_op_left_multiply_f", c_int32, [c_void_p, _DP, _DP]),
    ("ceres_hip_op_block_diagonal_ete", c_int32, [c_void_p, _DP, c_int64]),
    ("ceres_hip_op_block_diagonal_ftf", c_int32, [c_void_p, _DP, c_int64]),
    ("ceres_hip_op_squared_column_norm", c_int32, [c_void_p, _DP]),
    ("ceres_hip_op_jtjx", c_int32, [c_void_p, _DP, _DP]),
    ("ceres_hip_op_jtb", c_int32, [c_void_p, _DP]),
    ("ceres_hip_op_jacobian_gram", c_int32, [c_void_p, _DP, _DP, _DP]),
    ("ceres_hip_op_schur_init", c_int32, [c_void_p]),
    ("ceres_hip_get_schur_rhs", c_int32, [c_void_p, _DP]),
    ("ceres_hip_get_ete_inverse", c_int32, [c_void_p, _DP, c_int64]),
    ("ceres_hip_op_schur_sx", c_int32, [c_void_p, _DP, _DP]),
    ("ceres_hip_op_back_substitute", c_int32, [c_void_p, _DP, _DP]),
    ("ceres_hip_op_power_series_operator", c_int32, [c_void_p, _DP, _DP]),
    ("ceres_hip_op_spse_apply", c_int32, [c_void_p, _DP, _DP, c_int32, c_double]),
    ("ceres_hip_op_block_jacobi_update", c_int32, [c_void_p]),
    ("ceres_hip_op_schur_jacobi_update", c_int32, [c_void_p]),
    ("ceres_hip_op_cluster_jacobi_update", c_int32, [c_void_p]),
    ("ceres_hip_cluster_jacobi_stats", c_int32, [c_void_p, POINTER(c_int32), POINTER(c_int32), POINTER(c_int64), _DP]),
    ("ceres_hip_debug_cluster_cameras", c_int32, [POINTER(CBlockStructure), c_int32, c_int32, POINTER(c_int32), POINTER(c_int32)]),
    ("ceres_hip_get_preconditioner_blocks", c_int32, [c_void_p, c_int32, _DP, c_int64]),
    ("ceres_hip_op_precond_apply", c_int32, [c_void_p, _DP, _DP]),
    ("ceres_hip_op_schur_eliminate_dense", c_int32, [c_void_p, _DP, _DP]),
    ("ceres_hip_schur_storage_info", c_int32, [c_void_p, POINTER(c_int64), POINTER(c_int64)]),
# ... 266 lines not shown
            if not ok:
                self.p2p_error = self._lib.ceres_hip_last_error(self._h).decode()
            handles = p2p_exchange(bytes(mine))
            if len(handles) != world_size or any(len(h) != IPC_HANDLE_BYTES for h in handles):
                raise HipError("p2p_exchange must return one 64-byte handle per rank")
            if ok:
                allh = (c_uint8 * (IPC_HANDLE_BYTES * world_size)).from_buffer_copy(b"".join(handles))
                ok = self._lib.ceres_hip_comm_p2p_connect(self._h, allh) == 0
                if not ok:
                    self.p2p_error = self._lib.ceres_hip_last_error(self._h).decode()
            self.p2p_ok = ok
            if not ok and comm_id is None:
                raise HipError("peer-to-peer communicator failed and there is no RCCL communicator: " + self.p2p_error)
        if loopback_world > 1:
            self._check(self._lib.ceres_hip_debug_comm_loopback(self._h, loopback_world))
        if ghost_world > 1:
            self._check(self._lib.ceres_hip_debug_comm_ghost_peers(self._h, ghost_world, int(p2p_max_elements)))
            self.p2p_ok = True

    def p2p_selftest(self) -> bool:
        if not self.p2p_ok:
            return False
        rc = self._lib.ceres_hip_comm_p2p_selftest(self._h)
        if rc != 0:
            self.p2p_error = self._lib.ceres_hip_last_error(self._h).decode()
            self.p2p_ok = False
        return rc == 0

    def allreduce_timing(self, n: int, iters: int = 200) -> float:
        out = np.zeros(1)
        self._check(self._lib.ceres_hip_debug_allreduce_timing(self._h, int(n), int(iters), _p(out)))
        return float(out[0])

    def p2p_disable(self):
        self._check(self._lib.ceres_hip_comm_p2p_disable(self._h))
        self.p2p_ok = False

    def _check(self, rc):
        if rc != 0:
            raise HipError(f"ceres_hip error {rc}: {self._lib.ceres_hip_last_error(self._h).decode()}")

    def close(self):
        if getattr(self, "_h", None):
            self._lib.ceres_hip_destroy(self._h)
            self._h = None

    def __del__(self):
        try:
            self.close()
        except Exception:
            pass

    def __enter__(self):
        return self

    def __exit__(self, *exc):
        self.close()

    def set_structure(self, bs: BlockStructure):
        self.bs = bs
        self._cbs = bs.as_ctypes()
        self._check(self._lib.ceres_hip_set_structure(self._h, byref(self._cbs)))
        self._info = self.info()
        self._values_extent = bs.values_extent()

    def info(self) -> CInfo:
# ... 817 lines not shown
```

### include/ceres_hip.h

```cpp
#ifndef CERES_HIP_H_
#define CERES_HIP_H_

#include <stddef.h>
#include <stdint.h>

#ifdef __cplusplus
extern "C" {
#endif

#define CERES_HIP_ABI_VERSION 2

#define CERES_HIP_OK 0
#define CERES_HIP_E_INVALID (-1)
#define CERES_HIP_E_UNSUPPORTED (-2)
#define CERES_HIP_E_HIP (-3)
#define CERES_HIP_E_COMM (-4)
#define CERES_HIP_E_NODEVICE (-5)

#define CERES_HIP_DENSE_SCHUR 3
#define CERES_HIP_ITERATIVE_SCHUR 5
#define CERES_HIP_CGNR 6

#define CERES_HIP_IDENTITY 0
#define CERES_HIP_JACOBI 1
// ... 66 lines not shown
  int32_t p2p_enabled;
  int32_t p2p_fine_grained;
  int32_t camera_accum_hybrid;
  int32_t hybrid_popular_rows;
  int64_t num_observations_in_lds;
  int32_t points_renumbered;
  int32_t cg_iteration_in_operator;
  int32_t collectives_last_step;
} ceres_hip_info;

typedef struct ceres_hip_solver ceres_hip_solver;

int ceres_hip_abi_version(void);
int ceres_hip_device_count(void);
ceres_hip_solver* ceres_hip_create(const ceres_hip_options* options);
void ceres_hip_destroy(ceres_hip_solver* s);
const char* ceres_hip_last_error(const ceres_hip_solver* s);

int ceres_hip_set_structure(ceres_hip_solver* s, const ceres_hip_block_structure* bs);
int ceres_hip_get_info(const ceres_hip_solver* s, ceres_hip_info* info);

#define CERES_HIP_UNIQUE_ID_BYTES 128
int ceres_hip_comm_get_unique_id(uint8_t id[CERES_HIP_UNIQUE_ID_BYTES]);
int ceres_hip_comm_init(ceres_hip_solver* s, const uint8_t id[CERES_HIP_UNIQUE_ID_BYTES],
                        int32_t rank, int32_t world_size);

#define CERES_HIP_IPC_HANDLE_BYTES 64
int ceres_hip_comm_p2p_prepare(ceres_hip_solver* s, int32_t rank, int32_t world_size, int64_t max_elements,
                               uint8_t handle_out[CERES_HIP_IPC_HANDLE_BYTES]);
int ceres_hip_comm_p2p_connect(ceres_hip_solver* s, const uint8_t* all_handles );
int ceres_hip_comm_p2p_selftest(ceres_hip_solver* s);
int ceres_hip_comm_p2p_disable(ceres_hip_solver* s);
int ceres_hip_debug_allreduce_timing(ceres_hip_solver* s, int64_t n, int32_t iters, double* avg_us);

int ceres_hip_solve(ceres_hip_solver* s, const double* host_values, const double* host_b,
                    const double* host_D, double q_tolerance, double r_tolerance,
                    double* host_x, ceres_hip_summary* summary);
int ceres_hip_solve_unchanged_values(ceres_hip_solver* s, const double* host_D, double q_tolerance, double r_tolerance,
                                     double* host_x, ceres_hip_summary* summary);
int ceres_hip_solve_device(ceres_hip_solver* s, const double* dev_values, const double* dev_b,
                           const double* dev_D, double q_tolerance, double r_tolerance,
                           double* dev_x, ceres_hip_summary* summary);


int ceres_hip_load(ceres_hip_solver* s, const double* host_values, const double* host_b,
                   const double* host_D);
int ceres_hip_load_device(ceres_hip_solver* s, const double* dev_values, const double* dev_b,
                          const double* dev_D);

int ceres_hip_op_right_multiply(ceres_hip_solver* s, const double* x, double* y);
int ceres_hip_op_left_multiply(ceres_hip_solver* s, const double* x, double* y);
int ceres_hip_op_right_multiply_e(ceres_hip_solver* s, const double* x, double* y);
int ceres_hip_op_right_multiply_f(ceres_hip_solver* s, const double* x, double* y);
int ceres_hip_op_left_multiply_e(ceres_hip_solver* s, const double* x, double* y);
int ceres_hip_op_left_multiply_f(ceres_hip_solver* s, const double* x, double* y);
int ceres_hip_op_block_diagonal_ete(ceres_hip_solver* s, double* blocks, int64_t capacity);
int ceres_hip_op_block_diagonal_ftf(ceres_hip_solver* s, double* blocks, int64_t capacity);
int ceres_hip_op_squared_column_norm(ceres_hip_solver* s, double* x);
int ceres_hip_op_jtjx(ceres_hip_solver* s, const double* x, double* y);
int ceres_hip_op_jtb(ceres_hip_solver* s, double* y);
int ceres_hip_op_jacobian_gram(ceres_hip_solver* s, const double* a, const double* b, double* out);

int ceres_hip_op_schur_init(ceres_hip_solver* s);
int ceres_hip_get_schur_rhs(ceres_hip_solver* s, double* rhs);
int ceres_hip_get_ete_inverse(ceres_hip_solver* s, double* blocks, int64_t capacity);
int ceres_hip_op_schur_sx(ceres_hip_solver* s, const double* x, double* y);
// ... 292 lines not shown
```

Measured before the change: 712.0 steps/s.

## Replace back-substitution with point-tail recombination of captured CG point updates

During the fused Schur CG, each Sx pass now records the per-point E^T F p vectors and their alpha values for the first few iterations, and the init pass records E^T b. When CG finishes within that many updates, a lightweight point-wise kernel rebuilds the point solution (and the model cost) as Einv(etb - sum alpha_k u_k). This replaces the full Jacobian-streaming back-substitution pass. It costs extra HBM writes on every captured Sx pass, an extra u_hist buffer, and more complex routing logic. When CG runs longer than the cap, the solver falls back to ordinary back-substitution.

Result: faster. 773.8 steps/s (median of 6 runs) (+8.7%).

```diff
diff --git a/ceres-solver_amd/csrc/common.h b/ceres-solver_amd/csrc/common.h
--- a/ceres-solver_amd/csrc/common.h
+++ b/ceres-solver_amd/csrc/common.h
@@ -28,6 +28,7 @@
 constexpr int kStagedXMinTilesPerWg = 100;
 constexpr int kCamItemLaneMinMean = 384;
 constexpr int kCamItemSpread = 8192;
+constexpr int kPointTailMaxIterations = 4;
 constexpr int kNonTemporalTileMiB = 200;
 
 struct HostStructure {
diff --git a/ceres-solver_amd/csrc/device.h b/ceres-solver_amd/csrc/device.h
--- a/ceres-solver_amd/csrc/device.h
+++ b/ceres-solver_amd/csrc/device.h
@@ -121,6 +121,9 @@
   double* pq_out = nullptr;
   const int* status = nullptr;
   int* clear_flags = nullptr;
+  double* u_out = nullptr;
+  double* etb_out = nullptr;
+  const int* skip_updates = nullptr;
   CgTail tail;
 };
 
@@ -177,6 +180,24 @@
   int off[kMaxSharedScalars] = {}, width[kMaxSharedScalars] = {}, pos[kMaxSharedScalars] = {};
   int64_t out[kMaxSharedScalars] = {};
 };
+
+struct PointTailArgs {
+  int n_points = 0, n_f = 0;
+  const int32_t* pt_pos = nullptr;
+  const double* etei = nullptr;
+  const double* etb = nullptr;
+  const double* u_hist = nullptr;
+  int64_t u_stride = 0;
+  const double *D_e = nullptr, *D_f = nullptr;
+  const double *z = nullptr, *rhs = nullptr, *r = nullptr;
+  double *y_e = nullptr, *y_f = nullptr;
+  int negate = 0;
+  int* nonfinite = nullptr;
+  const CgScalars* S = nullptr;
+  double* cost_out = nullptr;
+};
+constexpr int kPointTailBlock = 256;
+constexpr int kPointTailMaxGrid = 1023;
 
 struct BalOps {
   int nr, ne, nf, ns, pairs, tile_pitch, cam_part, etei_pitch, b_pairs, mo_pitch, has_f32, has_cg_tail;
@@ -203,6 +224,7 @@
                               bool few );
   hipError_t (*camera_chunk)(const ZUnits& units, const double* ring, double* acc, const int* status, hipStream_t stream);
   hipError_t (*strip_finish)(const double* parts, int nparts, const StripBlocks& sb, const double* D_f, double* blocks, hipStream_t stream);
+  hipError_t (*point_tail)(const PointTailArgs& T, int* n_parts, hipStream_t stream);
 };
 const BalOps* GetBalOps(int nr, int ne, int nf, int ns);
 hipError_t AllowMaxLds(const void* kernel);
@@ -361,7 +383,13 @@
   int iter, status, min_it, max_it;
   int fail_dir, fail_step;
   double rho_pp[2], Q0_pp[2];
-};
+  double alpha_hist[kPointTailMaxIterations];
+  int n_updates, reserved;
+};
+__host__ __device__ inline bool PointTailTakes(int status, int updates) {
+  return (status == kCgConvergedZeta || status == kCgConvergedResidual || status == kCgMaxIterations) && updates >= 1 &&
+         updates <= kPointTailMaxIterations;
+}
 
 struct CgBuffers {
   int64_t n = 0;
diff --git a/ceres-solver_amd/csrc/kernels_bal.inc b/ceres-solver_amd/csrc/kernels_bal.inc
--- a/ceres-solver_amd/csrc/kernels_bal.inc
+++ b/ceres-solver_amd/csrc/kernels_bal.inc
@@ -763,6 +763,11 @@
   if (A.negate_out && !isfinite(t)) atomicAdd(A.nonfinite, 1);
 }
 
+__device__ __forceinline__ void store_point_capture(double* out, int po, const double* v) {
+#pragma unroll
+  for (int j = 0; j < NE; ++j) out[po + j] = v[j];
+}
+
 __device__ __forceinline__ double cost_terms(const double (&m)[NR], const double (&b)[NR], double half) {
   double t = 0.0;
 #pragma unroll
@@ -843,7 +848,7 @@
   }
 }
 
-template <int MODE, bool LDS>
+template <int MODE, bool LDS, int CAP = 0>
 __device__ __forceinline__ void compute_stream(const BalArgs& A, const Slot& s, int lane, int span, int npts,
                                                const StreamAux& x, Ctx& acc, double& dot) {
   if constexpr (MODE == kSx || MODE == kSpseZ) {
@@ -859,6 +864,25 @@
 #if !(CERES_HIP_AB_ABLATE & 4)
     seg_allreduce<NE>(u, lane, s.first, s.last, span);
 #endif
+    if constexpr (MODE == kSx && LDS && CAP == 1) {
+#if CERES_HIP_PIPELINED
+      const int n3 = 3 * npts;
+      double* const out = A.u_out + 3 * int64_t(__builtin_amdgcn_readfirstlane(s.pt));
+      const int ta = (s.seg >> 17) & 63, tb = (s.seg >> 24) & 63;
+      {
+        const double v0 = shfl_idx(u[0], ta), v1 = shfl_idx(u[1], ta), v2 = shfl_idx(u[2], ta);
+        const int c = lane % 3;
+        if ((s.seg >> 23) & 1) out[lane] = c == 0 ? v0 : (c == 1 ? v1 : v2);
+      }
+      if (n3 > 64) {
+        const double v0 = shfl_idx(u[0], tb), v1 = shfl_idx(u[1], tb), v2 = shfl_idx(u[2], tb);
+        const int c = (lane + 1) % 3;
+        if ((s.seg >> 30) & 1) out[64 + lane] = c == 0 ? v0 : (c == 1 ? v1 : v2);
+      }
+#endif
+    } else if constexpr (MODE == kSx && LDS && CAP == 0) {
+      if (A.u_out && s.valid && lane == s.last) store_point_capture(A.u_out, NE * s.pt, u);
+    }
     sym_mul(x.ei, u, v);
     double ev[NR], z[NR];
     e_times(s.e, v, ev);
@@ -1079,6 +1103,7 @@
     invert_spd_e(a, ei);
     if (s.valid && lane == s.last) store_ete_inverse(A, s.pt, ei);
     if constexpr (MODE == kInit) {
+      if (A.etb_out && s.valid && lane == s.last) store_point_capture(A.etb_out, po, r + kTriE);
       double g[NE];
 #pragma unroll
       for (int j = 0; j < NE; ++j) g[j] = r[kTriE + j];
@@ -1319,6 +1344,7 @@
       if (lane == 0) store_ete_inverse(A, pt, ei);
     }
     if constexpr (MODE == kInit) {
+      if (A.etb_out && lane == 0) store_point_capture(A.etb_out, po, r + kTriE);
       double g[NE];
 #pragma unroll
       for (int j = 0; j < NE; ++j) g[j] = r[kTriE + j];
@@ -1481,6 +1507,9 @@
       load_ete_inverse(A, pt, ei);
 #pragma unroll
       for (int j = 0; j < NE; ++j) u[j] = tot[j];
+      if constexpr (MODE == kSx && LDS) {
+        if (A.u_out && finish) store_point_capture(A.u_out, NE * pt, u);
+      }
       sym_mul(ei, u, v);
       if constexpr (MODE == kBackSub) {
         if (finish) store_point_solution(A, po, v);
@@ -1524,6 +1553,7 @@
         if (finish) store_ete_inverse(A, pt, ei);
       }
       if constexpr (MODE == kInit) {
+        if (A.etb_out && finish) store_point_capture(A.etb_out, po, tot + kTriE);
         if (apply) {
           double g[NE];
 #pragma unroll
@@ -1543,6 +1573,9 @@
   }
   if (A.status && *A.status != 0) return;
   if (A.run_after_cg && !CgStatusAllowsSolution(*A.run_after_cg)) return;
+  if constexpr (MODE == kBackSub) {
+    if (A.run_after_cg && A.skip_updates && PointTailTakes(*A.run_after_cg, *A.skip_updates)) return;
+  }
   constexpr bool kScatters = (MODE == kSx || MODE == kJtJx || MODE == kJtb || MODE == kInit || MODE == kCgnrInit || MODE == kColNorm || MODE == kSpseZ);
   Ctx acc;
   ctx_init(A, acc, nullptr);
@@ -1817,7 +1850,13 @@
     if (pq <= 0 || isinf(pq)) fail = kCgIndefinite;
     else { alpha = rho / pq; if (isinf(alpha)) fail = kCgFailAlpha; }
   }
-  if (threadIdx.x == 0) { S.pq = pq; S.alpha = alpha; S.rho_new = rho; S.fail_step = fail; }
+  if (threadIdx.x == 0) {
+    S.pq = pq; S.alpha = alpha; S.rho_new = rho; S.fail_step = fail;
+    if (!fail) {
+      if (it <= kPointTailMaxIterations) S.alpha_hist[it - 1] = alpha;
+      S.n_updates = it;
+    }
+  }
   if (fail) {
     if (threadIdx.x == 0) S.status = fail;
     return;
@@ -1887,7 +1926,7 @@
   }
 }
 
-template <int MODE, bool LDS>
+template <int MODE, bool LDS, bool CAP = false>
 __device__ __forceinline__ void compute_long_round(const BalArgs& A, const Slot& s, int lane, const StreamAux& x, uint32_t word, uint32_t word0,
                                                    int flag, int wave, double (*red)[3], double (&carry)[3], Ctx& acc, double& dot) {
   const bool active = word != kRoundIdle;
@@ -1898,6 +1937,7 @@
     f_times(s, acc, x.xc, t0, t1);
     double u[3] = {s.e[0] * t0 + s.e[3] * t1, s.e[1] * t0 + s.e[4] * t1, s.e[2] * t0 + s.e[5] * t1};
     if (!s.valid) { u[0] = u[1] = u[2] = 0; }
+    const int pt = __builtin_amdgcn_readfirstlane(s.pt);
     if (!(flag & kRoundApply)) {
       wave_allreduce<3>(u);
       if (lane == 0) { red[wave][0] = u[0]; red[wave][1] = u[1]; red[wave][2] = u[2]; }
@@ -1909,7 +1949,16 @@
     } else {
       u[0] = u[1] = u[2] = 0;
       for (int k = 0; k < cnt; ++k) { u[0] += red[w0 + k][0]; u[1] += red[w0 + k][1]; u[2] += red[w0 + k][2]; }
-      if (flag & kRoundSum) { carry[0] += u[0]; carry[1] += u[1]; carry[2] += u[2]; return; }
+      if (flag & kRoundSum) {
+        carry[0] += u[0]; carry[1] += u[1]; carry[2] += u[2];
+        if constexpr (MODE == kSx && LDS) {
+          if (CAP && (flag & kRoundLast) && active && wave == w0 && lane == 0) store_point_capture(A.u_out, NE * pt, carry);
+        }
+        return;
+      }
+      if constexpr (MODE == kSx && LDS) {
+        if (CAP && active && wave == w0 && lane == 0) store_point_capture(A.u_out, NE * pt, u);
+      }
     }
     double v[3];
     sym_mul(x.ei, u, v);
@@ -1950,7 +1999,7 @@
   }
 }
 
-template <int MODE, bool LDS, bool NT, bool F32 = false>
+template <int MODE, bool LDS, bool NT, bool F32 = false, bool CAP = false>
 __global__ __launch_bounds__(512) void bal_stream_kernel(BalArgs A) {
   constexpr int BLOCK = 512;
   extern __shared__ double lds_acc[];
@@ -2036,7 +2085,7 @@
       if (ckind != 0) c.valid = false;
       widen_slot<F32>(c);
       if constexpr (LDS) take_hot_x(A, c, xh, cx);
-      compute_stream<MODE, LDS>(A, c, lane, caux & 0xff, ckind == 0 ? caux >> 8 : 0, cx, acc, dot);
+      compute_stream<MODE, LDS, CAP ? 1 : 2>(A, c, lane, caux & 0xff, ckind == 0 ? caux >> 8 : 0, cx, acc, dot);
       __builtin_amdgcn_sched_barrier(0);
       i1 = i2;
       tile = min(tile + pstep, last);
@@ -2091,7 +2140,7 @@
       if (ckind != 0) c.valid = false;
       widen_slot<F32>(c);
       if constexpr (LDS) take_hot_x(A, c, xh, cx);
-      compute_stream<MODE, LDS>(A, c, lane, caux & 0xff, ckind == 0 ? caux >> 8 : 0, cx, acc, dot);
+      compute_stream<MODE, LDS, CAP ? 1 : 2>(A, c, lane, caux & 0xff, ckind == 0 ? caux >> 8 : 0, cx, acc, dot);
       __builtin_amdgcn_sched_barrier(0);
       i1 = i2;
       tile = next;
@@ -2167,7 +2216,7 @@
         __builtin_amdgcn_sched_barrier(0);
         widen_slot<F32>(c);
         if constexpr (LDS) take_hot_x(A, c, xh, cx);
-        compute_long_round<MODE, LDS>(A, c, lane, cx, cw, cw0, cf, wave, round_red[par], carry, acc, dot);
+        compute_long_round<MODE, LDS, CAP>(A, c, lane, cx, cw, cw0, cf, wave, round_red[par], carry, acc, dot);
         __builtin_amdgcn_sched_barrier(0);
         par ^= 1;
         i1 = i2;
@@ -3064,6 +3113,74 @@
   }
 }
 
+__global__ __launch_bounds__(kPointTailBlock) void bal_point_tail_kernel(PointTailArgs T) {
+  const int status = T.S->status, n = T.S->n_updates;
+  if (!PointTailTakes(status, n)) return;
+  double al[kPointTailMaxIterations];
+#pragma unroll
+  for (int k = 0; k < kPointTailMaxIterations; ++k) al[k] = k < n ? T.S->alpha_hist[k] : 0.0;
+  const double sg = T.negate ? -1.0 : 1.0;
+  const int64_t tid = int64_t(blockIdx.x) * kPointTailBlock + threadIdx.x, nthreads = int64_t(gridDim.x) * kPointTailBlock;
+  double cost = 0.0;
+  int bad = 0;
+  for (int64_t p = tid; p < T.n_points; p += nthreads) {
+    const int po = T.pt_pos ? T.pt_pos[p] : NE * int(p);
+    const double2* q = reinterpret_cast<const double2*>(T.etei + p * kEteiPitch);
+    double2 rec[kEteiPitch / 2];
+#pragma unroll
+    for (int j = 0; j < kEteiPitch / 2; ++j) rec[j] = q[j];
+    double ei[kTriE], U[NE], t[NE], w[NE], y[NE], eit[NE];
+#pragma unroll
+    for (int i = 0; i < kTriE; ++i) ei[i] = (i & 1) ? rec[i / 2].y : rec[i / 2].x;
+#pragma unroll
+    for (int j = 0; j < NE; ++j) { U[j] = 0.0; t[j] = T.etb[po + j]; }
+#pragma unroll
+    for (int k = 0; k < kPointTailMaxIterations; ++k) {
+      if (k < n) {
+#pragma unroll
+        for (int j = 0; j < NE; ++j) U[j] += al[k] * T.u_hist[k * T.u_stride + NE * p + j];
+      }
+    }
+#pragma unroll
+    for (int j = 0; j < NE; ++j) w[j] = t[j] - U[j];
+    sym_mul(ei, w, y);
+    double fin = 0.0;
+#pragma unroll
+    for (int j = 0; j < NE; ++j) { T.y_e[po + j] = sg * y[j]; fin += y[j]; }
+    if (!isfinite(fin)) ++bad;
+    if (T.cost_out) {
+      sym_mul(ei, t, eit);
+#pragma unroll
+      for (int j = 0; j < NE; ++j) {
+        const double d = T.D_e ? T.D_e[po + j] * y[j] : 0.0;
+        cost += y[j] * t[j] + U[j] * eit[j] + d * d;
+      }
+    }
+  }
+  for (int64_t i = tid; i < T.n_f; i += nthreads) {
+    const double z = T.z[i];
+    T.y_f[i] = sg * z;
+    if (!isfinite(z)) ++bad;
+    if (T.cost_out) {
+      const double d = T.D_f ? T.D_f[i] * z : 0.0;
+      cost += z * T.rhs[i] + z * T.r[i] + d * d;
+    }
+  }
+  if (bad && T.negate) atomicAdd(T.nonfinite, bad);
+  if (T.cost_out) {
+    __shared__ double red[kPointTailBlock / 64];
+#pragma unroll
+    for (int m = 32; m >= 1; m >>= 1) cost += __shfl_xor(cost, m, 64);
+    if ((threadIdx.x & 63) == 0) red[threadIdx.x >> 6] = cost;
+    __syncthreads();
+    if (threadIdx.x == 0) {
+      double s = 0.0;
+      for (int i = 0; i < kPointTailBlock / 64; ++i) s += red[i];
+      T.cost_out[blockIdx.x] = 0.5 * s;
+    }
+  }
+}
+
 }
 
 template <int MODE, int BLOCK, bool F32>
@@ -3095,10 +3212,10 @@
 }
 
 #if CERES_HIP_PIPELINED
-template <int MODE, bool NT, bool F32 = false>
+template <int MODE, bool NT, bool F32 = false, bool CAP = false>
 static hipError_t launch_stream2(const BalArgs& A, bool lds, int grid, hipStream_t stream) {
   if (lds) {
-    auto k = bal_stream_kernel<MODE, true, NT, F32>;
+    auto k = bal_stream_kernel<MODE, true, NT, F32, CAP>;
     if (hipError_t e = AllowMaxLds(reinterpret_cast<const void*>(k)); e != hipSuccess) return e;
     const size_t tail_bytes = (kHasCgTail && MODE == kSx && A.tail.enabled) ? size_t(512 + kCgTailMax) * sizeof(double) : 0;
     static const size_t static_lds = [&] { hipFuncAttributes fa{}; return hipFuncGetAttributes(&fa, reinterpret_cast<const void*>(k)) == hipSuccess ? size_t(fa.sharedSizeBytes) : size_t(1024); }();
@@ -3124,6 +3241,9 @@
     }
   }
   const bool nt = A.n_tiles * int64_t(kTilePitch) * int64_t(sizeof(double2)) > (int64_t(kNonTemporalTileMiB) << 20);
+  if constexpr (MODE == kSx) {
+    if (A.u_out && lds) return nt ? launch_stream2<MODE, true, false, true>(A, lds, grid, stream) : launch_stream2<MODE, false, false, true>(A, lds, grid, stream);
+  }
   return nt ? launch_stream2<MODE, true>(A, lds, grid, stream) : launch_stream2<MODE, false>(A, lds, grid, stream);
 }
 
@@ -3304,6 +3424,14 @@
   return hipGetLastError();
 }
 
+static hipError_t PointTail(const PointTailArgs& T, int* n_parts, hipStream_t stream) {
+  const int64_t work = std::max<int64_t>(T.n_points, T.n_f);
+  const int grid = int(std::max<int64_t>(1, std::min<int64_t>((work + kPointTailBlock - 1) / kPointTailBlock, kPointTailMaxGrid)));
+  if (n_parts) *n_parts = T.cost_out ? grid : 0;
+  hipLaunchKernelGGL(bal_point_tail_kernel, dim3(grid), dim3(kPointTailBlock), 0, stream, T);
+  return hipGetLastError();
+}
+
 }
 
 #define CERES_HIP_CAT2(a, b) a##b
@@ -3312,7 +3440,7 @@
   namespace sh = CERES_HIP_SHAPE;
   static const BalOps ops = {sh::NR, sh::NE, sh::NF, sh::NS, sh::kPairs, sh::kTilePitch, sh::kCamPart, sh::kEteiPitch, sh::kBPairs, sh::kMoPitch, sh::kHasF32 ? 1 : 0, sh::kHasCgTail ? 1 : 0,
                              sh::Fused, sh::SxRunsPipelined, sh::ReducePartials, sh::ReduceExchange, sh::StreamProbe, sh::AddFDiagonal, sh::Pack, sh::Invert, sh::CameraExchange,
-                             sh::CameraItems, sh::CameraFinish, sh::CameraChunk, sh::StripFinish};
+                             sh::CameraItems, sh::CameraFinish, sh::CameraChunk, sh::StripFinish, sh::PointTail};
   return &ops;
 }
 
diff --git a/ceres-solver_amd/csrc/kernels_cg.hip b/ceres-solver_amd/csrc/kernels_cg.hip
--- a/ceres-solver_amd/csrc/kernels_cg.hip
+++ b/ceres-solver_amd/csrc/kernels_cg.hip
@@ -165,7 +165,7 @@
     S.Q1 = 0; S.zeta = 0; S.norm_r = S.norm_rhs; S.norm_p = 0; S.norm_q = 0;
     S.iter = 1; S.min_it = min_it; S.max_it = max_it;
     S.status = kCgRunning;
-    S.fail_dir = 0; S.fail_step = 0;
+    S.fail_dir = 0; S.fail_step = 0; S.n_updates = 0;
     if (S.norm_rhs == 0.0) S.status = kCgZeroRhs;
     else if (min_it == 0 && S.norm_r <= S.tol_r) S.status = kCgInitialResidual;
     if (B.setup_fail && *B.setup_fail != 0) S.status = kCgSetupFailed;
@@ -209,7 +209,7 @@
   S.Q0_pp[0] = Q0; S.Q0_pp[1] = Q0; S.rho_pp[0] = 1.0; S.rho_pp[1] = 1.0;
   S.iter = 1; S.min_it = min_it; S.max_it = max_it;
   S.status = kCgRunning;
-  S.fail_dir = 0; S.fail_step = 0;
+  S.fail_dir = 0; S.fail_step = 0; S.n_updates = 0;
   if (S.norm_rhs == 0.0) S.status = kCgZeroRhs;
   else if (min_it == 0 && S.norm_r <= S.tol_r) S.status = kCgInitialResidual;
   if (B.setup_fail && *B.setup_fail != 0) S.status = kCgSetupFailed;
@@ -508,6 +508,10 @@
     S.alpha = alpha;
     S.rho_new = rho;
     S.fail_step = fail;
+    if (!fail) {
+      if (it <= kPointTailMaxIterations) S.alpha_hist[it - 1] = alpha;
+      S.n_updates = it;
+    }
   }
 }
 
@@ -536,7 +540,7 @@
     S.Q0 = 0.0; S.Q1 = 0; S.zeta = 0; S.norm_r = norm_rhs; S.norm_p = 0; S.norm_q = 0;
     S.Q0_pp[0] = 0.0; S.Q0_pp[1] = 0.0; S.rho_pp[0] = 1.0; S.rho_pp[1] = rho;
     S.iter = 1; S.min_it = min_it; S.max_it = max_it;
-    S.fail_dir = fail_dir; S.fail_step = 0;
+    S.fail_dir = fail_dir; S.fail_step = 0; S.n_updates = 0;
     S.status = status;
   }
 }
diff --git a/ceres-solver_amd/csrc/solver.hip b/ceres-solver_amd/csrc/solver.hip
--- a/ceres-solver_amd/csrc/solver.hip
+++ b/ceres-solver_amd/csrc/solver.hip
@@ -97,6 +97,17 @@
   bool spec_tail_done = false;
   int spec_cgnr_parts = 0;
   int backsub_cost_parts = 0;
+  bool point_tail = true;
+  bool point_tail_eligible = false;
+  double* d_u_hist = nullptr;
+  double* d_etb = nullptr;
+  bool pt_tail_armed = false;
+  int cg_capture_it = 0;
+  int cg_enqueued = 0;
+  bool pt_tail_enqueued = false, backsub_enqueued = false;
+  bool backsub_skips_for_tail = false;
+  int pt_tail_parts = 0;
+  int last_backsub_route = 0;
   bool lm_fuse_active = false;
   ceres_hip_lm_options lm_opts{};
   double* d_camsq = nullptr;
@@ -563,6 +574,11 @@
   return 0;
 }
 
+double* point_tail_capture(const ceres_hip_solver* s, const double* x) {
+  if (s->cg_capture_it < 1 || s->cg_capture_it > kPointTailMaxIterations || x != s->cg.p || !s->d_u_hist) return nullptr;
+  return s->d_u_hist + size_t(s->cg_capture_it - 1) * size_t(s->hs.num_cols_e);
+}
+
 int op_sx(ceres_hip_solver* s, const double* x, double* y, const int* status, double* pq = nullptr, int* n_pq = nullptr) {
   const HostStructure& h = s->hs;
   if (n_pq) *n_pq = 0;
@@ -570,6 +586,7 @@
     TRY(ensure_packed(s));
     BalArgs A = bal_args(s);
     A.x_f = x;
+    A.u_out = point_tail_capture(s, x);
     return bal_scatter(s, kBalSx, A, x, y, true, status, pq, n_pq);
   }
   const double* v = s->values;
@@ -657,6 +674,7 @@
     BalArgs A = bal_args(s);
     A.D_e = s->D;
     A.Mo = want_Mo ? s->d_Mo : nullptr;
+    if (s->point_tail_eligible && s->have_b) A.etb_out = s->d_etb;
     if (s->clear_flags_pending) { A.clear_flags = s->d_nonfinite; s->clear_flags_pending = false; }
     PackGuard g = use_gather_if_unpacked(s, A);
     if (s->have_b) {
@@ -702,7 +720,10 @@
     s->backsub_cost_parts = 0;
     if (s->lm_want_model_cost && z != nullptr) { A.scalar_out = s->scalar_partials; s->backsub_cost_parts = s->fused_grid; }
     if (h.num_cols_f > 0 && z != nullptr) { A.copy_src = z; A.copy_dst = x + h.num_cols_e; A.copy_n = h.num_cols_f; }
-    if (s->gate_on_cg_status) A.run_after_cg = &s->cg.S->status;
+    if (s->gate_on_cg_status) {
+      A.run_after_cg = &s->cg.S->status;
+      if (s->backsub_skips_for_tail) A.skip_updates = &s->cg.S->n_updates;
+    }
     if (s->lm_negate_in_solve && z != nullptr) {
       if (!s->nonfinite_clean) HIP_TRY(s, hipMemsetAsync(s->d_nonfinite, 0, sizeof(int), st));
       s->nonfinite_clean = false;
@@ -1034,6 +1055,23 @@
   *dev_parts = s->cg.comm;
   return 0;
 }
+int op_point_tail(ceres_hip_solver* s, const double* z, double* x) {
+  const HostStructure& h = s->hs;
+  PointTailArgs T;
+  T.n_points = s->plan.n_points; T.n_f = h.num_cols_f;
+  T.pt_pos = s->plan.points_contiguous ? nullptr : s->d_pt_pos;
+  T.etei = s->etei; T.etb = s->d_etb; T.u_hist = s->d_u_hist; T.u_stride = h.num_cols_e;
+  T.D_e = s->D; T.D_f = s->D ? s->D + h.num_cols_e : nullptr;
+  T.z = z; T.rhs = s->rhs_f; T.r = s->cg.r;
+  T.y_e = x; T.y_f = x + h.num_cols_e;
+  T.negate = s->lm_negate_in_solve ? 1 : 0;
+  T.nonfinite = s->d_nonfinite;
+  T.S = s->cg.S;
+  T.cost_out = s->lm_want_model_cost ? s->scalar_partials : nullptr;
+  HIP_TRY(s, s->ops->point_tail(T, &s->pt_tail_parts, s->stream));
+  return 0;
+}
+
 struct CgSpec {
   int64_t n = 0;
   int64_t n_local = 0;
@@ -1190,6 +1228,9 @@
   s->h_scalars->status = kCgRunning;
   s->timing.operator_applications = 0;
   int it = 1;
+  const bool capture = s->pt_tail_armed && fused_start;
+  s->pt_tail_armed = capture;
+  struct CaptureOff { ceres_hip_solver* s; ~CaptureOff() { s->cg_capture_it = 0; } } capture_off{s};
   auto precondition = [&]() -> int {
     if (spec.precondition) {
       TRY(spec.precondition(B.r, B.z));
@@ -1209,6 +1250,7 @@
     const int batch_end = std::min(max_it, it + interval - 1);
     for (; it <= batch_end; ++it) {
       const int reset = (it % reset_period == 0) ? 1 : 0;
+      s->cg_capture_it = (capture && it <= kPointTailMaxIterations) ? it : 0;
       if (fused && spec.iteration && !reset) {
         const int done = spec.iteration(it);
         if (done < 0) return CERES_HIP_E_HIP;
@@ -1255,6 +1297,8 @@
       TRY(collapse_and_reduce(s, 2, 2));
       HIP_TRY(s, LaunchCgFinalize(B, st));
     }
+    s->cg_capture_it = 0;
+    s->cg_enqueued = it - 1;
     if (spec.before_poll) TRY(spec.before_poll());
     TRY(poll_scalars(s));
     if (adaptive) { interval = first_batch ? 2 : std::min(16, interval * 2); first_batch = false; }
@@ -1641,6 +1685,7 @@
         if (!s->ops->sx_runs_pipelined(A)) return 0;
         CgBuffers& B = s->cg;
         A.x_f = B.p;
+        A.u_out = point_tail_capture(s, B.p);
         A.status = status;
         A.tail.enabled = 1; A.tail.it = it; A.tail.ticket = s->d_cg_ticket;
         A.tail.x = B.x; A.tail.r = B.r; A.tail.p = B.p; A.tail.z = B.z; A.tail.rhs = B.rhs;
@@ -1662,11 +1707,30 @@
       spec.x0_nonzero = true;
     }
     s->spec_tail_done = false;
+    s->pt_tail_armed = s->point_tail_eligible && s->have_b && !spec.x0_nonzero && !spec.precondition && h.num_cols_f > 0;
+    s->pt_tail_enqueued = s->backsub_enqueued = false;
+    s->last_backsub_route = 0;
     if (s->lm_speculate && s->path == CERES_HIP_PATH_BAL && h.num_cols_f > 0) {
       spec.before_poll = [s, x]() {
-        s->gate_on_cg_status = true;
-        const int rc = op_back_substitute(s, s->cg.x, x);
-        s->gate_on_cg_status = false;
+        int rc = 0;
+        s->pt_tail_enqueued = s->pt_tail_armed;
+        s->backsub_enqueued = !s->pt_tail_armed || s->cg_enqueued > kPointTailMaxIterations;
+        if (s->pt_tail_enqueued) {
+          if (s->lm_negate_in_solve) {
+            if (!s->nonfinite_clean) HIP_TRY(s, hipMemsetAsync(s->d_nonfinite, 0, sizeof(int), s->stream));
+            s->nonfinite_clean = s->backsub_enqueued;
+            s->lm_negated = true;
+          }
+          rc = op_point_tail(s, s->cg.x, x);
+          if (rc) return rc;
+        }
+        if (s->backsub_enqueued) {
+          s->gate_on_cg_status = true;
+          s->backsub_skips_for_tail = s->pt_tail_enqueued;
+          rc = op_back_substitute(s, s->cg.x, x);
+          s->gate_on_cg_status = false;
+          s->backsub_skips_for_tail = false;
+        }
         if (rc) return rc;
         if (s->world > 1) {
           if (s->mailbox && s->d_h_pinned) {
@@ -1683,10 +1747,35 @@
         return 0;
       };
     }
-    TRY(run_cg(s, spec, q_tol, r_tol, summary));
+    const int rc_cg = run_cg(s, spec, q_tol, r_tol, summary);
+    const bool armed = s->pt_tail_armed;
+    s->pt_tail_armed = false;
+    TRY(rc_cg);
     TRY(rec(s, 5));
-    if (summary->termination_type != CERES_HIP_FAILURE && summary->termination_type != CERES_HIP_FATAL_ERROR && !s->spec_tail_done)
-      TRY(op_back_substitute(s, s->cg.x, x));
+    const bool usable = summary->termination_type != CERES_HIP_FAILURE && summary->termination_type != CERES_HIP_FATAL_ERROR;
+    const bool tail_takes = armed && PointTailTakes(s->h_scalars->status, s->h_scalars->n_updates);
+    if (s->spec_tail_done) {
+      if (s->pt_tail_enqueued && tail_takes) {
+        s->last_backsub_route = 1;
+        s->backsub_cost_parts = s->pt_tail_parts;
+      } else if (!s->backsub_enqueued && usable) {
+        s->spec_tail_done = false;
+        TRY(op_back_substitute(s, s->cg.x, x));
+      }
+    } else if (usable) {
+      if (tail_takes) {
+        if (s->lm_negate_in_solve) {
+          if (!s->nonfinite_clean) HIP_TRY(s, hipMemsetAsync(s->d_nonfinite, 0, sizeof(int), s->stream));
+          s->nonfinite_clean = false;
+          s->lm_negated = true;
+        }
+        TRY(op_point_tail(s, s->cg.x, x));
+        s->last_backsub_route = 1;
+        s->backsub_cost_parts = s->pt_tail_parts;
+      } else {
+        TRY(op_back_substitute(s, s->cg.x, x));
+      }
+    }
     TRY(rec(s, 6));
     return 0;
   }
@@ -2099,6 +2188,9 @@
   TRY(dev_alloc(s, &s->cg_pq_parts, size_t(kMaxPqParts)));
   { const char* e = getenv("CERES_HIP_CG_FUSED"); s->cg_fused = !(e && atoi(e) == 0); }
   { const char* e = getenv("CERES_HIP_SPECULATE"); s->speculate = !(e && atoi(e) == 0); }
+  { const char* e = getenv("CERES_HIP_POINT_TAIL"); s->point_tail = !(e && atoi(e) == 0); }
+  s->point_tail_eligible = false;
+  s->d_u_hist = s->d_etb = nullptr;
   s->cg.S = reinterpret_cast<CgScalars*>(s->scalar_partials + kScalarsOffset);
   HIP_TRY(s, hipMemsetAsync(s->cg.S, 0, sizeof(CgScalars), s->stream));
   TRY(dev_alloc(s, &s->precond, size_t(is_schur(s) ? h.diag_off_f.back() : h.diag_off_all.back()) + 2 * size_t(h.num_cols_f)));
@@ -2198,6 +2290,15 @@
       s->chunk_grid = P.hybrid ? P.hyb_groups : int(std::max<int64_t>(1, std::min<int64_t>(s->num_cus, (chunk_tiles + 15) / 16)));
     }
     TRY(dev_alloc(s, &s->d_camsq, n9));
+    s->point_tail_eligible = s->point_tail && s->opt.solver_type == CERES_HIP_ITERATIVE_SCHUR && !s->opt.use_explicit_schur_complement &&
+                             !is_cluster_jacobi(s) && s->opt.preconditioner_type != CERES_HIP_SCHUR_POWER_SERIES_EXPANSION && s->cg_fused &&
+                             s->world <= 1 && s->lds_mode && P.n_rem_rows == 0 && P.ns == 0 && s->opt.jacobian_storage != 1 &&
+                             h.num_cols_e > 0 && h.num_cols_f > 0 && s->ops->point_tail != nullptr &&
+                             P.long_behind && P.n_tiles < (int64_t(1) << 26);
+    if (s->point_tail_eligible) {
+      TRY(dev_alloc(s, &s->d_u_hist, size_t(kPointTailMaxIterations) * size_t(h.num_cols_e)));
+      TRY(dev_alloc(s, &s->d_etb, size_t(h.num_cols_e)));
+    }
     if (P.ns > 0) TRY(dev_alloc(s, &s->d_strip_parts, size_t(s->fused_grid) * size_t(P.ns * (P.ns + 1) / 2)));
     if (s->cgnr_internal) TRY(dev_alloc(s, &s->D_int, size_t(h.num_cols_e)));
     if (s->world > 1 && (is_schur(s) ? (P.cameras_contiguous && P.cam_base == 0) : P.caller_contiguous) && int64_t(n9) == int64_t(h.num_cols_f)) {
diff --git a/ceres-solver_amd/csrc/solver_debug.inc b/ceres-solver_amd/csrc/solver_debug.inc
--- a/ceres-solver_amd/csrc/solver_debug.inc
+++ b/ceres-solver_amd/csrc/solver_debug.inc
@@ -1,3 +1,5 @@
+
+int ceres_hip_debug_last_backsub_route(const ceres_hip_solver* s) { return s ? s->last_backsub_route : CERES_HIP_E_INVALID; }
 
 int ceres_hip_debug_staged_x_plan(const ceres_hip_block_structure* bs, int32_t num_eliminate_blocks, int64_t counts[4], int32_t* staged_cam,
                                   int32_t* slot_word, int64_t staged_capacity, int64_t slot_capacity) {
diff --git a/ceres-solver_amd/hip_solver.py b/ceres-solver_amd/hip_solver.py
--- a/ceres-solver_amd/hip_solver.py
+++ b/ceres-solver_amd/hip_solver.py
@@ -89,6 +89,7 @@
     ("ceres_hip_comm_p2p_selftest", c_int32, [c_void_p]),
     ("ceres_hip_comm_p2p_disable", c_int32, [c_void_p]),
     ("ceres_hip_debug_allreduce_timing", c_int32, [c_void_p, c_int64, c_int32, _DP]),
+    ("ceres_hip_debug_last_backsub_route", c_int32, [c_void_p]),
     ("ceres_hip_solve", c_int32, [c_void_p, _DP, _DP, _DP, c_double, c_double, _DP, POINTER(CSummary)]),
     ("ceres_hip_solve_device", c_int32, [c_void_p, c_void_p, c_void_p, c_void_p, c_double, c_double, c_void_p, POINTER(CSummary)]),
     ("ceres_hip_solve_unchanged_values", c_int32, [c_void_p, _DP, c_double, c_double, _DP, POINTER(CSummary)]),
@@ -421,6 +422,9 @@
         self._check(self._lib.ceres_hip_debug_allreduce_timing(self._h, int(n), int(iters), _p(out)))
         return float(out[0])
 
+    def last_backsub_route(self) -> int:
+        return int(self._lib.ceres_hip_debug_last_backsub_route(self._h))
+
     def p2p_disable(self):
         self._check(self._lib.ceres_hip_comm_p2p_disable(self._h))
         self.p2p_ok = False
diff --git a/include/ceres_hip.h b/include/ceres_hip.h
--- a/include/ceres_hip.h
+++ b/include/ceres_hip.h
@@ -122,6 +122,7 @@
 int ceres_hip_comm_p2p_selftest(ceres_hip_solver* s);
 int ceres_hip_comm_p2p_disable(ceres_hip_solver* s);
 int ceres_hip_debug_allreduce_timing(ceres_hip_solver* s, int64_t n, int32_t iters, double* avg_us);
+int ceres_hip_debug_last_backsub_route(const ceres_hip_solver* s);
 
 int ceres_hip_solve(ceres_hip_solver* s, const double* host_values, const double* host_b,
                     const double* host_D, double q_tolerance, double r_tolerance,
```
